# jeff-regier/Celeste.jl

Measured on AMD Instinct MI355X. Metric: sources/sec (ELBO value+gradient+Hessian+KL per target source), higher is better.
Workload: dtype f64; 1 GPU; BASELINE.json configs[2]: synthetic 2048x1489x5 SDSS-size field, 2000 star+galaxy sources, fp64, Sa=1 with value-only neighbours, psf_K=2; gather_backend=none, neighbor_links_rank0=3526

## Files before the change

### __graft_entry__.py

```python
import os
import subprocess
import sys

ROOT = os.path.dirname(os.path.abspath(__file__))
CSRC = os.path.join(ROOT, "celeste.jl_amd", "csrc")
LIB = os.path.join(CSRC, "libceleste_mi355x.so")
HIPCC = os.environ.get("HIPCC", "/opt/rocm/bin/hipcc")
HIP_FLAGS = ["--offload-arch=gfx950", "-O3", "-std=c++17", "-fPIC", "-shared", "-Wl,--version-script=exports.map"]
LINK_FLAGS = ["-L/opt/rocm/lib", "-lrccl", "-lpthread"]
DETECT_DIR = os.path.join(CSRC, "detect")
DETECT_LIB = os.path.join(DETECT_DIR, "libceleste_detect.so")
MCMC_DIR = os.path.join(CSRC, "mcmc")
MCMC_LIB = os.path.join(MCMC_DIR, "libceleste_mcmc.so")
BLEND_DIR = os.path.join(CSRC, "blend")
BLEND_LIB = os.path.join(BLEND_DIR, "libceleste_blend.so")
SYNTH_DIR = os.path.join(CSRC, "synth")
SYNTH_LIB = os.path.join(SYNTH_DIR, "libceleste_synth.so")


def _stale(target, sources):
    if not os.path.exists(target):
        return True
    t = os.path.getmtime(target)
    return any(os.path.getmtime(s) > t for s in sources)


def build() -> None:
    srcs = [os.path.join(CSRC, f) for f in os.listdir(CSRC) if f.endswith((".hip", ".h", ".inc", ".map"))]
    srcs.append(os.path.join(ROOT, "include", "celeste_mi355x.h"))
    srcs.append(os.path.abspath(__file__))
    if _stale(LIB, srcs):
        subprocess.check_call([HIPCC] + HIP_FLAGS + ["-o", LIB, os.path.join(CSRC, "celeste_abi.hip")] + LINK_FLAGS, cwd=CSRC)
    dsrcs = [os.path.join(DETECT_DIR, f) for f in os.listdir(DETECT_DIR) if f.endswith((".hip", ".h", ".map"))]
    dsrcs += [os.path.join(ROOT, "include", "celeste_detect.h"), os.path.abspath(__file__)]
    if _stale(DETECT_LIB, dsrcs):
        subprocess.check_call([HIPCC] + HIP_FLAGS + ["-o", DETECT_LIB, os.path.join(DETECT_DIR, "celeste_detect.hip"), "-lpthread"],
                              cwd=DETECT_DIR)
    msrcs = [os.path.join(MCMC_DIR, f) for f in os.listdir(MCMC_DIR) if f.endswith((".hip", ".h", ".map"))]
    msrcs += [os.path.join(CSRC, f) for f in os.listdir(CSRC) if f.endswith((".h", ".inc"))]
    msrcs += [os.path.join(ROOT, "include", "celeste_mcmc.h"), os.path.join(ROOT, "include", "celeste_mi355x.h"),
              os.path.abspath(__file__)]
    if _stale(MCMC_LIB, msrcs):
        subprocess.check_call([HIPCC] + HIP_FLAGS + ["-o", MCMC_LIB, os.path.join(MCMC_DIR, "celeste_mcmc.hip"), "-lpthread"],
                              cwd=MCMC_DIR)
    bsrcs = [os.path.join(BLEND_DIR, f) for f in os.listdir(BLEND_DIR) if f.endswith((".hip", ".h", ".map"))]
    bsrcs += [os.path.join(CSRC, f) for f in os.listdir(CSRC) if f.endswith((".hip", ".h", ".inc"))]
    bsrcs += [os.path.join(ROOT, "include", "celeste_blend.h"), os.path.join(ROOT, "include", "celeste_mi355x.h"),
              os.path.abspath(__file__)]
    if _stale(BLEND_LIB, bsrcs):
        subprocess.check_call([HIPCC] + HIP_FLAGS + ["-o", BLEND_LIB, os.path.join(BLEND_DIR, "celeste_blend.hip")] + LINK_FLAGS,
                              cwd=BLEND_DIR)
    ssrcs = [os.path.join(SYNTH_DIR, f) for f in os.listdir(SYNTH_DIR) if f.endswith((".hip", ".h", ".map"))]
    ssrcs += [os.path.join(CSRC, f) for f in os.listdir(CSRC) if f.endswith((".h", ".inc"))]
    ssrcs += [os.path.join(ROOT, "include", "celeste_synth.h"), os.path.join(ROOT, "include", "celeste_mi355x.h"),
              os.path.abspath(__file__)]
    if _stale(SYNTH_LIB, ssrcs):
        subprocess.check_call([HIPCC] + HIP_FLAGS + ["-o", SYNTH_LIB, os.path.join(SYNTH_DIR, "celeste_synth.hip"), "-lpthread"],
                              cwd=SYNTH_DIR)
    subprocess.check_call(["make", "-s", "-C", os.path.join(ROOT, "oracle")])
    fake_src, fake_lib = os.path.join(ROOT, "tests", "fake_rccl.c"), os.path.join(ROOT, "tests", "libfake_rccl.so")
    if _stale(fake_lib, [fake_src]):
        subprocess.check_call(["gcc", "-O2", "-fPIC", "-shared", "-Wall", "-D__HIP_PLATFORM_AMD__", "-I/opt/rocm/include", fake_src, "-o", fake_lib,
                               "-L/opt/rocm/lib", "-lamdhip64", "-lpthread", "-Wl,-rpath,/opt/rocm/lib"])
    if ROOT not in sys.path:
        sys.path.insert(0, ROOT)
    import celeste_jl_amd
    from celeste_jl_amd import cabi
    lib = cabi.load_library()
    for name in cabi.EXPORTED_SYMBOLS:
        getattr(lib, name)
    from celeste_jl_amd import detect
    dlib = detect.load_library()
    for name in detect.EXPORTED_SYMBOLS:
        getattr(dlib, name)
    from celeste_jl_amd import mcmc
    mlib = mcmc.load_library()
    for name in mcmc.EXPORTED_SYMBOLS:
        getattr(mlib, name)
    from celeste_jl_amd import blend
    blib = blend.load_library()
    for name in blend.EXPORTED_SYMBOLS:
        getattr(blib, name)
    from celeste_jl_amd import synth
    slib = synth.load_library()
    for name in synth.EXPORTED_SYMBOLS:
        getattr(slib, name)


def smoke() -> None:
    if ROOT not in sys.path:
        sys.path.insert(0, ROOT)
    import numpy as np
    import celeste_jl_amd as cel
    from celeste_jl_amd import synthetic, cabi
    from oracle import oracle
    f = synthetic.make_sample_dataset("two_body", seed=1)
    ctx = cel.FieldContext(f.images, f.patches, f.neighbors)
    v, d, h, cnt, st = ctx.eval_batch(f.vp, [0, 1])
    ov, od, oh, ocnt, ost = oracle.elbo_batch(ctx.problem, f.vp, [0, 1], n_threads=1)
    assert (st == 0).all() and (ost == 0).all()
    assert np.array_equal(cnt, ocnt), (cnt, ocnt)
    for a, b, name in ((v, ov, "v"), (d, od, "d"), (h, oh, "h")):
        scale = np.abs(b).max()
        err = np.abs(a - b).max() / scale
        assert err < 1e-8, (name, err)
    print("smoke ok: elbo =", v, "max rel err vs oracle < 1e-8")


if __name__ == "__main__":
    build()
    if len(sys.argv) > 1 and sys.argv[1] == "smoke":
        smoke()
```

### celeste.jl_amd/cabi.py

```python
import ctypes as C
import os
from typing import List, Optional, Sequence

import numpy as np

P = 44
STAMP = 51
COEF = 53

OK, ERR_INVALID_ARG, ERR_NONFINITE_INPUT, ERR_NONFINITE_RESULT, ERR_HIP, ERR_NO_DEVICE, ERR_ALLOC, ERR_ABORTED = range(8)
FLAG_GRAD, FLAG_HESS, FLAG_KL, FLAG_FP32, FLAG_SPLIT, FLAG_PACKED_HESS = 1, 2, 4, 8, 16, 32
HP = 990

_HERE = os.path.dirname(os.path.abspath(__file__))
LIB_PATH = os.path.join(_HERE, "csrc", "libceleste_mi355x.so")

c_double_p = C.POINTER(C.c_double)
c_float_p = C.POINTER(C.c_float)
c_int32_p = C.POINTER(C.c_int32)
c_int64_p = C.POINTER(C.c_int64)
c_uint8_p = C.POINTER(C.c_uint8)


class ImageT(C.Structure):
    _fields_ = [("H", C.c_int32), ("W", C.c_int32), ("band", C.c_int32), ("reserved", C.c_int32),
                ("pixels", c_float_p), ("sky", c_float_p), ("nelec_per_nmgy", c_float_p)]


class PatchT(C.Structure):
    _fields_ = [("off_h", C.c_int32), ("off_w", C.c_int32), ("H2", C.c_int32), ("W2", C.c_int32),
                ("bitmap", c_uint8_p), ("wcs_jacobian", C.c_double * 4), ("world_center", C.c_double * 2),
                ("pixel_center", C.c_double * 2), ("psf", c_double_p), ("stamp", C.c_int32),
                ("reserved", C.c_int32)]


class PriorT(C.Structure):
    _fields_ = [("is_star", C.c_double * 2), ("flux_mean", C.c_double * 2), ("flux_var", C.c_double * 2),
                ("k", (C.c_double * 8) * 2), ("color_mean", ((C.c_double * 4) * 8) * 2),
                ("color_cov", ((C.c_double * 16) * 8) * 2), ("gal_radius_px_mean", C.c_double),
                ("gal_radius_px_var", C.c_double)]


class ProblemT(C.Structure):
    _fields_ = [("n_images", C.c_int32), ("n_sources", C.c_int32), ("psf_K", C.c_int32), ("n_stamps", C.c_int32),
                ("images", C.POINTER(ImageT)), ("patches", C.POINTER(PatchT)), ("stamps", c_double_p),
                ("nbr_offsets", c_int64_p), ("nbr_index", c_int32_p), ("prior", C.POINTER(PriorT)),
                ("n_patch_entries", C.c_int64), ("patch_source", c_int32_p), ("patch_image", c_int32_p)]


class WorkStatsT(C.Structure):
    _fields_ = [("n_targets", C.c_int64), ("active_pixel_visits", C.c_int64), ("patch_rows", C.c_int64),
                ("neighbor_links", C.c_int64), ("algorithmic_bytes", C.c_int64), ("record_bytes", C.c_int64),
                ("record_tiles", C.c_int64)]


class OptimConfigT(C.Structure):
    _fields_ = [("loc_width", C.c_double), ("loc_scale", C.c_double), ("max_iters", C.c_int32),
                ("include_kl", C.c_int32), ("xtol_abs", C.c_double), ("ftol_rel", C.c_double), ("gtol", C.c_double),
                ("initial_delta", C.c_double), ("delta_hat", C.c_double), ("tr_secular_iters", C.c_int32),
                ("reserved", C.c_int32)]


class GroupInfoT(C.Structure):
    _fields_ = [("n_members", C.c_int32), ("n_devices", C.c_int32), ("exchange", C.c_int32), ("rccl_ranks", C.c_int32),
                ("devices", C.c_int32 * 16)]


EXCHANGE_RCCL, EXCHANGE_PEER_COPY = 1, 2


class CelesteError(RuntimeError):
    def __init__(self, status: int, msg: str):
        super().__init__("celeste_mi355x status %d: %s" % (status, msg))
        self.status = status


EXPORTED_SYMBOLS = [
    "celeste_version", "celeste_strerror", "celeste_ctx_create", "celeste_ctx_destroy", "celeste_elbo_eval",
    "celeste_elbo_eval_batch", "celeste_elbo_eval_multi", "celeste_elbo_eval_batch_device", "celeste_ctx_enable_timing",
    "celeste_ctx_last_kernel_ms", "celeste_ctx_last_record_sum_ms", "celeste_ctx_work_stats", "celeste_spline_prefilter",
    "celeste_ctx_spline_coefficients", "celeste_psf_raster",
    "celeste_maximize_batch", "celeste_render_expected", "celeste_optim_stats", "celeste_tr_solve_batch",
    "celeste_images_create", "celeste_images_destroy", "celeste_ctx_create_on",
    "celeste_host_alloc", "celeste_host_free", "celeste_host_register", "celeste_host_unregister",
    "celeste_maximize_batch_device", "celeste_joint_infer",
    "celeste_group_create", "celeste_group_destroy", "celeste_group_info", "celeste_group_elbo_eval_batch",
    "celeste_group_sweep_plan", "celeste_group_sweep", "celeste_group_sweep_wait", "celeste_group_sweep_results",
    "celeste_group_shard_sizes", "celeste_group_enable_timing", "celeste_group_last_sweep_ms", "celeste_group_last_kernel_ms",
    "celeste_group_maximize_batch", "celeste_group_joint_infer", "celeste_group_collectives",
]
ABI_VERSION = 220

_lib = None


def load_library(path: Optional[str] = None) -> C.CDLL:
    global _lib
    if _lib is not None and path is None:
        return _lib
    path = path or os.environ.get("CELESTE_MI355X_LIB") or LIB_PATH
    if not os.path.exists(path):
        raise ImportError(
            "HIP extension %s is missing: build it with `python -c 'import __graft_entry__ as g; g.build()'` "
            "(hipcc --offload-arch=gfx950). There is no CPU fallback." % path)
    try:
        import torch
        if torch.cuda.is_available():
            torch.cuda.init()
    except ImportError:
        pass
    except RuntimeError:
        pass
    lib = C.CDLL(path)
    vp = C.c_void_p
    lib.celeste_version.restype = C.c_int
    if lib.celeste_version() // 100 != ABI_VERSION // 100:
        raise ImportError("%s has ABI version %d, this binding was written against %d: the struct layouts "
                          "(celeste_optim_config_t ...) may differ -- rebuild the library" % (path, lib.celeste_version(), ABI_VERSION))
    lib.celeste_strerror.restype = C.c_char_p
    lib.celeste_strerror.argtypes = [C.c_int]
    lib.celeste_ctx_create.argtypes = [C.POINTER(ProblemT), C.c_int, C.POINTER(vp)]
    lib.celeste_ctx_destroy.argtypes = [vp]
    lib.celeste_ctx_destroy.restype = None
    lib.celeste_elbo_eval.argtypes = [vp, c_double_p, C.c_int32, C.c_uint32, c_double_p, c_double_p, c_double_p,
                                      c_int64_p, c_int64_p]
    lib.celeste_elbo_eval_batch.argtypes = [vp, c_double_p, C.c_int32, c_int32_p, C.c_uint32, c_double_p,
                                            c_double_p, c_double_p, c_int64_p, c_int32_p]
    lib.celeste_elbo_eval_batch_device.argtypes = [vp, vp, C.c_int32, vp, C.c_uint32, vp, vp, vp, vp, vp, vp]
    lib.celeste_ctx_enable_timing.argtypes = [vp, C.c_int]
    lib.celeste_ctx_last_kernel_ms.argtypes = [vp, C.POINTER(C.c_float)]
    lib.celeste_elbo_eval_multi.argtypes = [vp, c_double_p, C.c_int32, c_int32_p, C.c_uint32, C.POINTER(C.c_double),
                                            c_double_p, c_double_p, C.POINTER(C.c_int64), C.POINTER(C.c_int64)]
    lib.celeste_ctx_last_record_sum_ms.argtypes = [vp, C.POINTER(C.c_float)]
    lib.celeste_ctx_work_stats.argtypes = [vp, C.c_int32, c_int32_p, C.POINTER(WorkStatsT)]
    lib.celeste_spline_prefilter.argtypes = [c_double_p, c_double_p]
    lib.celeste_ctx_spline_coefficients.argtypes = [vp, C.c_int32, c_double_p]
    lib.celeste_psf_raster.argtypes = [C.c_int, c_double_p, C.c_int32, c_double_p, C.c_int32, c_double_p,
                                       C.c_int32, c_double_p]
    lib.celeste_maximize_batch.argtypes = [vp, c_double_p, c_double_p, c_double_p, C.c_int32, c_int32_p,
                                           C.POINTER(OptimConfigT), c_int32_p, c_int32_p, c_double_p, c_int32_p]
    lib.celeste_maximize_batch_device.argtypes = [vp, vp, vp, vp, C.c_int32, vp, C.POINTER(OptimConfigT), vp, vp, vp, vp, vp]
    lib.celeste_joint_infer.argtypes = [vp, c_double_p, C.c_int32, c_int64_p, c_int32_p, c_double_p,
                                        C.POINTER(OptimConfigT), c_int32_p, c_int32_p, c_double_p, c_int32_p]
    lib.celeste_optim_stats.argtypes = [C.c_int, C.POINTER(C.c_uint64)]
    lib.celeste_tr_solve_batch.argtypes = [C.c_int, C.c_int32, c_double_p, c_double_p, c_double_p, C.c_int32, C.c_int32,
                                           c_double_p, c_double_p, c_int32_p, c_int32_p]
    lib.celeste_render_expected.argtypes = [vp, c_double_p, C.c_int32, c_double_p]
    lib.celeste_images_create.argtypes = [C.c_int32, C.POINTER(ImageT), C.c_int, C.POINTER(vp)]
    lib.celeste_images_destroy.argtypes = [vp]
    lib.celeste_images_destroy.restype = None
    lib.celeste_ctx_create_on.argtypes = [vp, C.POINTER(ProblemT), C.POINTER(vp)]
    lib.celeste_host_alloc.argtypes = [C.c_size_t]
    lib.celeste_host_alloc.restype = vp
    lib.celeste_host_free.argtypes = [vp]
    lib.celeste_host_free.restype = None
    lib.celeste_host_register.argtypes = [vp, C.c_size_t]
    lib.celeste_host_unregister.argtypes = [vp]
    c_float_p_ = C.POINTER(C.c_float)
    lib.celeste_group_create.argtypes = [C.POINTER(ProblemT), C.c_int32, c_int32_p, C.POINTER(vp)]
    lib.celeste_group_destroy.argtypes = [vp]
    lib.celeste_group_destroy.restype = None
    lib.celeste_group_info.argtypes = [vp, C.POINTER(GroupInfoT)]
    lib.celeste_group_collectives.argtypes = [vp, c_int64_p, c_int32_p]
    lib.celeste_group_elbo_eval_batch.argtypes = [vp, c_double_p, C.c_int32, c_int32_p, C.c_uint32, c_double_p, c_double_p,
                                                  c_double_p, c_int64_p, c_int32_p]
    lib.celeste_group_sweep_plan.argtypes = [vp, c_double_p, C.c_int32, c_int32_p, C.c_uint32]
    lib.celeste_group_sweep.argtypes = [vp]
    lib.celeste_group_sweep_wait.argtypes = [vp]
    lib.celeste_group_sweep_results.argtypes = [vp, c_double_p, c_double_p, c_double_p, c_int64_p, c_int32_p]
    lib.celeste_group_shard_sizes.argtypes = [vp, c_int32_p, c_int64_p]
    lib.celeste_group_enable_timing.argtypes = [vp, C.c_int]
    lib.celeste_group_last_sweep_ms.argtypes = [vp, c_float_p_, c_float_p_]
    lib.celeste_group_last_kernel_ms.argtypes = [vp, C.c_int32, c_float_p_]
    lib.celeste_group_maximize_batch.argtypes = [vp, c_double_p, c_double_p, c_double_p, C.c_int32, c_int32_p,
                                                 C.POINTER(OptimConfigT), c_int32_p, c_int32_p, c_double_p, c_int32_p]
    lib.celeste_group_joint_infer.argtypes = [vp, c_double_p, C.c_int32, C.c_int32, c_int64_p, c_int64_p, c_int32_p, c_double_p,
                                              C.POINTER(OptimConfigT), c_int32_p, c_int32_p, c_double_p, c_int32_p, c_int64_p]
    _lib = lib
    return lib


def check(status: int, lib=None):
    if status != OK:
        lib = lib or load_library()
        raise CelesteError(status, lib.celeste_strerror(status).decode())


def _dp(a: np.ndarray):
    return a.ctypes.data_as(c_double_p)


def marshal_image_structs(images, keep: list):
    c_images = (ImageT * len(images))()
    for n, im in enumerate(images):
        pix = np.asfortranarray(im.pixels, dtype=np.float32)
        sky = np.asfortranarray(im.sky, dtype=np.float32)
        iota = np.ascontiguousarray(im.nelec_per_nmgy, dtype=np.float32)
        assert sky.shape == pix.shape and iota.shape == (pix.shape[0],)
        keep += [pix, sky, iota]
        ci = c_images[n]
        ci.H, ci.W, ci.band = pix.shape[0], pix.shape[1], int(im.b)
        ci.pixels = pix.ctypes.data_as(c_float_p)
        ci.sky = sky.ctypes.data_as(c_float_p)
        ci.nelec_per_nmgy = iota.ctypes.data_as(c_float_p)
    return c_images


class ImageSet:

    def __init__(self, images, device: int = 0):
        self.lib = load_library()
# ... 288 lines not shown
```

### celeste.jl_amd/csrc/celeste_abi.hip

```cpp
#include <hip/hip_runtime.h>
#include <algorithm>
#include <atomic>
#include <cmath>
#include <cstdio>
#include <cstdlib>
#include <cstring>
#include <mutex>
#include <unordered_map>
#include <vector>

#include "elbo_kernels.h"
#include "optim_kernels.h"
#include "fused_kernels.h"
#include "host_tables.h"

struct celeste_group;

#define EVAL_FUSED_MAX 32

#define HIP_TRY(expr)                                                                    \
    do {                                                                                 \
        hipError_t e__ = (expr);                                                         \
        if (e__ != hipSuccess) {                                                         \
            fprintf(stderr, "celeste_mi355x: %s failed: %s (%s:%d)\n", #expr,            \
// ... 49 lines not shown
    static const size_t cap = [] { const char *v = getenv("CELESTE_PINNED_POOL_KB"); return (size_t)(v ? std::max(0, atoi(v)) : 16384) << 10; }();
    return cap;
}
static hipError_t staging_alloc(void **p, size_t bytes) {
    *p = nullptr;
    int k = -1;
    if (pinned_pool_cap() && bytes <= (1u << 20)) { k = 0; while (((size_t)4096 << k) < bytes) ++k; }
    if (k < 0) return hipHostMalloc(p, std::max<size_t>(bytes, 1), hipHostMallocPortable);
    PinnedPool &pp = pinned_pool();
    {
        std::lock_guard<std::mutex> lk(pp.mu);
        if (!pp.idle[k].empty()) { *p = pp.idle[k].back(); pp.idle[k].pop_back(); pp.idle_bytes -= (size_t)4096 << k; pp.live[*p] = k; return hipSuccess; }
    }
    hipError_t e = hipHostMalloc(p, (size_t)4096 << k, hipHostMallocPortable);
    if (e == hipSuccess) { std::lock_guard<std::mutex> lk(pp.mu); pp.live[*p] = k; }
    return e;
}
static void staging_free(void *p) {
    if (!p) return;
    {
        PinnedPool &pp = pinned_pool();
        std::lock_guard<std::mutex> lk(pp.mu);
        auto it = pp.live.find(p);
        if (it != pp.live.end()) {
            const int k = it->second;
            pp.live.erase(it);
            if (pp.idle_bytes + ((size_t)4096 << k) <= pinned_pool_cap()) { pp.idle[k].push_back(p); pp.idle_bytes += (size_t)4096 << k; return; }
        }
    }
    (void)hipHostFree(p);
}


struct celeste_images {
    int device = 0;
    int N = 0;
    std::vector<DevImage> h_images;
    std::vector<void *> plane_allocs;
    DevImage *d_images = nullptr;
    std::atomic<int> refs{1};
};

static void images_release(celeste_images *im) {
    if (!im || im->refs.fetch_sub(1) != 1) return;
    (void)hipSetDevice(im->device);
    for (void *p : im->plane_allocs) (void)hipFree(p);
    if (im->d_images) (void)hipFree(im->d_images);
    delete im;
}

struct celeste_ctx {
    int device = 0;
    celeste_images *imgs = nullptr;
    hipStream_t stream = nullptr;
    hipStream_t copy_stream = nullptr;
    bool copy_stream_checked = false;
    int N = 0, S = 0, K = 0, NC = 0, n_stamps = 0;
    int chunk_px = 256, CH = 1;
    int max_npx = 0;
    std::vector<DevPatch> h_patches;
    std::vector<int64_t> h_nbr_off;
    std::vector<int32_t> h_nbr_idx;
    DevImage *d_images = nullptr;
    DevPatch *d_patches = nullptr;
    double *d_coefs = nullptr;
    float *d_coefs_f = nullptr;
    uint8_t *d_bitmaps = nullptr;
    int64_t *d_nbr_off = nullptr;
    int32_t *d_nbr_idx = nullptr;
    PriorDev *d_prior = nullptr;
    SrcImg *d_srcimg = nullptr;
    Comp *d_comps = nullptr;
    SrcGeo *d_geo = nullptr;
    int64_t *d_val_off = nullptr;
    double2 *d_val = nullptr;
    int32_t *d_needed = nullptr;
    int32_t stamp = 0;
    std::vector<int32_t> h_vis_off, h_vis_img, h_vis_src;
    int32_t *d_vis_off = nullptr, *d_vis_img = nullptr, *d_vis_src = nullptr;
    int4 *d_value_items = nullptr;
    int4 *d_vitems_src = nullptr;
    int32_t *d_vitem_off = nullptr;
    std::vector<int32_t> h_vitem_off;
    int64_t n_value_items = 0;
    int32_t *d_prep_mark = nullptr;
    double *d_lg_sum = nullptr;
    int64_t *d_nv_base = nullptr;
    int32_t *d_nbr_vis = nullptr;
    int2 *d_items = nullptr;
    size_t items_cap = 0;
    std::vector<int32_t> h_src_chunks;
    std::vector<int64_t> h_top_chunks;
    int max_src_chunks = 0;
    int32_t *d_work = nullptr, *d_work_blk = nullptr, *d_work_total = nullptr;
    size_t work_cap = 0, work_blk_cap = 0;
    int M = 1;
    bool dense = false;
    int64_t V = 0;
    std::vector<int64_t> h_tile_off;
    int64_t *d_tile_off = nullptr;
    int64_t n_tiles = 0;
    int sum_tiles = 4, RCH = 1;
    double *d_rec = nullptr;
    double *d_acc_split = nullptr;
    size_t acc_split_cap = 0;
    double *d_acc = nullptr;
    size_t acc_cap = 0;
    int32_t *d_rec_off = nullptr;
    size_t rec_off_cap = 0;
    double *d_vp = nullptr;
    int32_t *d_targets = nullptr;
    double *d_v = nullptr, *d_d = nullptr, *d_h = nullptr;
    int64_t *d_cnt = nullptr;
    int32_t *d_status = nullptr;
    size_t stage_cap = 0;
    double *p_vp = nullptr;
    int32_t *p_targets = nullptr, *p_status = nullptr;
    double *p_v = nullptr, *p_d = nullptr, *p_h = nullptr;
    int64_t *p_cnt = nullptr;
    size_t pin_cap = 0;
    double *d_small_in = nullptr, *p_small_in = nullptr, *d_small_out = nullptr, *p_small_out = nullptr;
    static const int MAX_PARTS = 8;
    hipEvent_t part_done[MAX_PARTS] = {}, part_copied[MAX_PARTS] = {};
    struct OptBuffers {
        size_t cap = 0;
        double *d_vp = nullptr, *d_v = nullptr, *d_d = nullptr, *d_h = nullptr, *d_H = nullptr, *d_T = nullptr, *d_S = nullptr, *d_pos = nullptr;
        int32_t *d_targets = nullptr, *d_act[2] = {nullptr, nullptr}, *d_evt[2] = {nullptr, nullptr}, *d_count = nullptr,
                *d_st = nullptr;
        void *d_state = nullptr;
        static const int RING = 4;
        double *h_vp = nullptr;
        void *h_state = nullptr;
        int32_t *h_count = nullptr;
        hipEvent_t ev[RING] = {};
    } opt;
    struct FusedBuffers {
        size_t cap_t = 0, cap_rec = 0, cap_q = 0, cap_saved = 0;
        bool arrivals_dirty = true;
        int4 *d_chunk_desc = nullptr;
        int2 *d_tgt_rec = nullptr;
        int32_t *d_q_items = nullptr, *d_q_ctl = nullptr, *d_arrivals = nullptr;
        double *d_saved = nullptr;
        int32_t *h_ctl = nullptr;
        int max_resident = 0;
        int cus = 0;
    } fused;
    struct Scratch { void *p = nullptr; size_t cap = 0; } scratch[24];
    int timing = 0;
    hipEvent_t ev[5] = {nullptr, nullptr, nullptr, nullptr, nullptr};
    int ev_split = 0;
    int ev_valid = 0;
};

#define ABI_CATCH catch (const std::bad_alloc &) { return CELESTE_ERR_ALLOC; } catch (...) { return CELESTE_ERR_HIP; }

extern "C" int celeste_version(void) { return CELESTE_ABI_VERSION; }

extern "C" const char *celeste_strerror(int status) {
    switch (status) {
        case CELESTE_OK: return "ok";
        case CELESTE_ERR_INVALID_ARG: return "invalid argument";
        case CELESTE_ERR_NONFINITE_INPUT: return "vp contains NaNs or Infs";
        case CELESTE_ERR_NONFINITE_RESULT: return "ELBO value, gradient or Hessian contains Inf/NaNs";
        case CELESTE_ERR_HIP: return "HIP runtime error";
        case CELESTE_ERR_NO_DEVICE: return "no HIP device (the engine has no CPU fallback)";
        case CELESTE_ERR_ALLOC: return "allocation failed";
        case CELESTE_ERR_ABORTED: return "device group aborted: a member failed in front of a collective (destroy the group and create it again)";
// ... 277 lines not shown
        CTX_TRY(dev_upload(&c->d_val_off, voff.data(), voff.size()));
        CTX_TRY(dev_upload<double2>(&c->d_val, nullptr, (size_t)tot));
        CTX_TRY(dev_upload<int32_t>(&c->d_needed, nullptr, (size_t)c->S));
        if (hipMemset(c->d_needed, 0, (size_t)c->S * sizeof(int32_t)) != hipSuccess) { celeste_ctx_destroy(c); return CELESTE_ERR_HIP; }
    }

    CTX_TRY(dev_upload(&c->d_vis_off, c->h_vis_off.data(), c->h_vis_off.size()));
    CTX_TRY(dev_upload(&c->d_vis_img, c->h_vis_img.data(), c->h_vis_img.size()));
    CTX_TRY(dev_upload(&c->d_vis_src, c->h_vis_src.data(), c->h_vis_src.size()));
    CTX_TRY(dev_upload<double>(&c->d_lg_sum, nullptr, (size_t)c->V));
    if (c->V > 0)
        hipLaunchKernelGGL(patch_lgamma_kernel, dim3((unsigned)c->V), dim3(256), 0, nullptr, c->d_images, c->d_patches,
                           c->d_vis_img, c->d_bitmaps, c->d_lg_sum);
    const char *env_chunk = getenv("CELESTE_CHUNK_PX");
    if (env_chunk && atoi(env_chunk) >= 64) c->chunk_px = (atoi(env_chunk) + 63) / 64 * 64;
    c->CH = c->max_npx > 0 ? (c->max_npx + c->chunk_px - 1) / c->chunk_px : 1;
    c->h_src_chunks.assign((size_t)c->S, 0);
    for (int s = 0; s < c->S; ++s) {
        for (int v = c->h_vis_off[s]; v < c->h_vis_off[s + 1]; ++v) {
            const DevPatch &q = c->h_patches[v];
            c->h_src_chunks[s] += (q.H2 * q.W2 + c->chunk_px - 1) / c->chunk_px;
        }
        c->max_src_chunks = std::max(c->max_src_chunks, c->h_src_chunks[s]);
    }
    auto hv = [c](int s, int n) -> int64_t {
        if (c->dense) return (int64_t)s * c->N + n;
        const int32_t *b = c->h_vis_img.data() + c->h_vis_off[s], *e = c->h_vis_img.data() + c->h_vis_off[s + 1];
        const int32_t *it = std::lower_bound(b, e, n);
        return it != e && *it == n ? (int64_t)(it - c->h_vis_img.data()) : -1;
    };
    if (!c->dense) {
        std::vector<int64_t> base((size_t)c->S + 1, 0);
        for (int s = 0; s < c->S; ++s)
            base[s + 1] = base[s] + (int64_t)(c->h_vis_off[s + 1] - c->h_vis_off[s]) * (c->h_nbr_off[s + 1] - c->h_nbr_off[s]);
        std::vector<int32_t> nv((size_t)base[c->S]);
        for (int s = 0; s < c->S; ++s) {
            const int64_t K = c->h_nbr_off[s + 1] - c->h_nbr_off[s];
            for (int v = c->h_vis_off[s]; v < c->h_vis_off[s + 1]; ++v)
                for (int64_t q = 0; q < K; ++q)
                    nv[base[s] + (int64_t)(v - c->h_vis_off[s]) * K + q] = (int32_t)hv(c->h_nbr_idx[c->h_nbr_off[s] + q], c->h_vis_img[v]);
        }
        CTX_TRY(dev_upload(&c->d_nv_base, base.data(), base.size()));
        CTX_TRY(dev_upload(&c->d_nbr_vis, nv.data(), nv.size()));
    }
    {
        std::vector<int32_t> sorted(c->h_src_chunks);
        std::sort(sorted.begin(), sorted.end(), [](int32_t a, int32_t b) { return a > b; });
        c->h_top_chunks.assign((size_t)c->S + 1, 0);
        for (int s = 0; s < c->S; ++s) c->h_top_chunks[s + 1] = c->h_top_chunks[s] + sorted[s];
    }
    CTX_TRY(dev_upload<int32_t>(&c->d_work_total, nullptr, 1));
    {
        if (c->N > 0xffff) { celeste_ctx_destroy(c); return CELESTE_ERR_INVALID_ARG; }
        const int n_cls = c->chunk_px / 64;
        std::vector<std::vector<std::pair<int32_t, int32_t>>> by_len(n_cls);
        for (int s = 0; s < c->S; ++s)
            for (int64_t q = c->h_nbr_off[s]; q < c->h_nbr_off[s + 1]; ++q) {
                const int s2 = c->h_nbr_idx[q];
                for (int va = c->h_vis_off[s]; va < c->h_vis_off[s + 1]; ++va) {
                    const int n = c->h_vis_img[va];
                    const int64_t vb = hv(s2, n);
                    if (vb < 0) continue;
                    const DevPatch &a = c->h_patches[va], &b = c->h_patches[vb];
                    const int rh = std::min(a.off_h + a.H2, b.off_h + b.H2) - std::max(a.off_h, b.off_h);
                    const int rw = std::min(a.off_w + a.W2, b.off_w + b.W2 - 1) - std::max(a.off_w, b.off_w);
                    if (rh <= 0 || rw <= 0) continue;
                    const int npx = rh * rw, nch = (npx + c->chunk_px - 1) / c->chunk_px;
                    for (int ch = 0; ch < nch; ++ch) {
                        const int px = std::min(c->chunk_px, npx - ch * c->chunk_px);
                        by_len[n_cls - (px + 63) / 64].push_back({(int32_t)q, (int32_t)(n | (ch << 16))});
                    }
                }
            }
        std::vector<int32_t> link_src(c->h_nbr_idx.size());
        for (int s = 0; s < c->S; ++s)
            for (int64_t q = c->h_nbr_off[s]; q < c->h_nbr_off[s + 1]; ++q) link_src[q] = s;
        std::vector<int4> desc;
        for (auto &v : by_len)
            for (auto &e : v) {
                const int t = link_src[e.first], s2 = c->h_nbr_idx[e.first], n = e.second & 0xffff, ch = e.second >> 16;
                desc.push_back(make_int4((int)hv(s2, n), (int)hv(t, n), ch, t));
            }
        c->n_value_items = (int64_t)desc.size();
        CTX_TRY(dev_upload(&c->d_value_items, desc.data(), desc.size()));
        c->h_vitem_off.assign((size_t)c->S + 1, 0);
        for (auto &d : desc) c->h_vitem_off[(size_t)d.w + 1]++;
        for (int s = 0; s < c->S; ++s) c->h_vitem_off[s + 1] += c->h_vitem_off[s];
        {
            std::vector<int4> by_src(desc.size());
            std::vector<int32_t> fill(c->h_vitem_off.begin(), c->h_vitem_off.end() - 1);
            for (auto &d : desc) by_src[(size_t)fill[d.w]++] = d;
            CTX_TRY(dev_upload(&c->d_vitems_src, by_src.data(), by_src.size()));
            CTX_TRY(dev_upload(&c->d_vitem_off, c->h_vitem_off.data(), c->h_vitem_off.size()));
        }
        CTX_TRY(dev_upload<int32_t>(&c->d_prep_mark, nullptr, (size_t)c->S));
        if (hipMemset(c->d_prep_mark, 0, (size_t)c->S * sizeof(int32_t)) != hipSuccess) { celeste_ctx_destroy(c); return CELESTE_ERR_HIP; }
    }
    {
        c->h_tile_off.resize(c->h_patches.size());
        int64_t tot = 0;
        for (size_t q = 0; q < c->h_patches.size(); ++q) {
            c->h_tile_off[q] = tot;
            tot += ((int64_t)c->h_patches[q].H2 * c->h_patches[q].W2 + 63) / 64;
        }
        c->n_tiles = tot;
        if (const char *e = getenv("CELESTE_SUM_TILES")) if (atoi(e) > 0) c->sum_tiles = atoi(e);
        c->RCH = std::max(1, ((c->max_npx + 63) / 64 + c->sum_tiles - 1) / c->sum_tiles);
    }
    if (hipStreamSynchronize(nullptr) != hipSuccess) { celeste_ctx_destroy(c); return CELESTE_ERR_HIP; }
#undef CTX_TRY
    *out = c;
    return CELESTE_OK;
} ABI_CATCH

extern "C" void celeste_ctx_destroy(celeste_ctx_t *c) {
    if (!c) return;
    (void)hipSetDevice(c->device);
    if (c->stream) (void)hipStreamSynchronize(c->stream);
    if (c->copy_stream) (void)hipStreamSynchronize(c->copy_stream);
    void *ptrs[] = {c->d_patches, c->d_coefs, c->d_coefs_f, c->d_bitmaps, c->d_nbr_off, c->d_nbr_idx, c->d_prior,
                    c->d_srcimg, c->d_comps, c->d_geo, c->d_val_off, c->d_val, c->d_needed, c->d_vis_off, c->d_vis_img, c->d_vis_src, c->d_value_items, c->d_vitems_src, c->d_vitem_off, c->d_prep_mark, c->d_rec_off, c->d_lg_sum, c->d_nv_base, c->d_nbr_vis, c->d_items, c->d_work, c->d_work_blk, c->d_work_total, c->d_tile_off, c->d_rec, c->d_acc_split, c->d_acc, c->d_vp, c->d_targets, c->d_v, c->d_d, c->d_h,
                    c->d_cnt, c->d_status};
    for (void *p : ptrs) if (p) (void)hipFree(p);
    {
        auto &o = c->opt;
        void *optr[] = {o.d_vp, o.d_v, o.d_d, o.d_h, o.d_H, o.d_T, o.d_S, o.d_pos, o.d_targets, o.d_act[0], o.d_act[1], o.d_evt[0], o.d_evt[1],
                        o.d_count, o.d_st, o.d_state};
        for (void *q : optr) if (q) (void)hipFree(q);
        void *hptr[] = {o.h_vp, o.h_state, o.h_count};
        for (void *q : hptr) if (q) staging_free(q);
        for (int k = 0; k < celeste_ctx::OptBuffers::RING; ++k) if (o.ev[k]) (void)hipEventDestroy(o.ev[k]);
        auto &f = c->fused;
        void *fptr[] = {f.d_chunk_desc, f.d_tgt_rec, f.d_q_items, f.d_q_ctl, f.d_arrivals, f.d_saved};
        for (void *q : fptr) if (q) (void)hipFree(q);
        if (f.h_ctl) staging_free(f.h_ctl);
    }
    for (auto &sc : c->scratch) if (sc.p) (void)hipFree(sc.p);
    for (int i = 0; i < 5; ++i) if (c->ev[i]) (void)hipEventDestroy(c->ev[i]);
    for (int i = 0; i < celeste_ctx::MAX_PARTS; ++i) {
        if (c->part_done[i]) (void)hipEventDestroy(c->part_done[i]);
        if (c->part_copied[i]) (void)hipEventDestroy(c->part_copied[i]);
    }
    void *pins[] = {c->p_vp, c->p_targets, c->p_status, c->p_v, c->p_d, c->p_h, c->p_cnt, c->p_small_in, c->p_small_out};
    if (c->d_small_in) (void)hipFree(c->d_small_in);
    if (c->d_small_out) (void)hipFree(c->d_small_out);
    for (void *q : pins) if (q) staging_free(q);
    stream_retire(c->device, c->stream);
    stream_retire(c->device, c->copy_stream);
    images_release(c->imgs);
    delete c;
}

template <class T>
static hipError_t scratch_get(celeste_ctx_t *c, int k, size_t bytes, T **out) {
    auto &s = c->scratch[k];
    if (bytes > s.cap) {
        hipError_t e = s.p ? hipStreamSynchronize(c->stream) : hipSuccess;
        if (e != hipSuccess) return e;
        if (s.p) { (void)hipFree(s.p); s.p = nullptr; s.cap = 0; }
        e = hipMalloc(&s.p, std::max<size_t>(bytes, 256));
        if (e != hipSuccess) return e;
        s.cap = std::max<size_t>(bytes, 256);
    }
    *out = (T *)s.p;
    return hipSuccess;
}

static int launch_eval(celeste_ctx_t *c, const double *d_vp, int32_t n_targets, const int32_t *d_targets,
                       uint32_t flags, double *d_v, double *d_d, double *d_h, int64_t *d_counters, int32_t *d_status,
                       void *stream_, bool render_neighbors, const int32_t *d_active_rank = nullptr,
                       int64_t n_chunks = -1, bool tables_current = false, const int32_t *d_live = nullptr,
                       bool prep_all = false, bool render_only = false, const int32_t *d_h_pos = nullptr);

extern "C" int celeste_elbo_eval_batch_device(celeste_ctx_t *c, const double *d_vp, int32_t n_targets,
                                              const int32_t *d_targets, uint32_t flags, double *d_v, double *d_d,
                                              double *d_h, int64_t *d_counters, int32_t *d_status, void *stream_) try {
    return launch_eval(c, d_vp, n_targets, d_targets, flags, d_v, d_d, d_h, d_counters, d_status, stream_, true);
} ABI_CATCH

static int ensure_part_events(celeste_ctx_t *c, int n) {
    for (int k = 0; k < n && k < celeste_ctx::MAX_PARTS; ++k) {
        if (!c->part_done[k]) HIP_TRY(hipEventCreateWithFlags(&c->part_done[k], hipEventDisableTiming));
        if (!c->part_copied[k]) HIP_TRY(hipEventCreateWithFlags(&c->part_copied[k], hipEventDisableTiming));
    }
    return CELESTE_OK;
}

static void fused_args_tables(celeste_ctx_t *c, FusedArgs &A) {
    A.images = c->d_images; A.patches = c->d_patches; A.coefs = c->d_coefs; A.bitmaps = c->d_bitmaps;
    A.nbr_off = c->d_nbr_off; A.nbr_idx = c->d_nbr_idx; A.val_off = c->d_val_off; A.val = c->d_val;
    A.nv_base = c->d_nv_base; A.nbr_vis = c->d_nbr_vis; A.items = c->dense ? nullptr : c->d_items; A.geo = c->d_geo;
    A.prior = c->d_prior; A.vis_off = c->d_vis_off; A.vis_img = c->d_vis_img; A.lg_sum = c->d_lg_sum; A.rec_off = c->d_rec_off;
    A.N = c->N; A.NC = c->NC; A.K = c->K; A.M = c->M; A.CH = c->CH; A.chunk_px = c->chunk_px;
    A.acc = c->d_acc;
    A.st = nullptr; A.Hstate = nullptr; A.Tstate = nullptr; A.Spec = nullptr; A.q_items = nullptr; A.q_ctl = nullptr; A.q_cap = 0; A.timeout_ticks = 0;
    A.j_R = 0; A.j_gshift = 0; A.j_dep = nullptr; A.j_succ_off = nullptr; A.j_succ = nullptr; A.j_vitem_off = nullptr;
    A.j_vitems = nullptr; A.j_render_arr = nullptr; A.j_saved = nullptr; A.j_pos = nullptr; A.j_srcimg = nullptr;
    A.j_comps = nullptr; A.j_geo = nullptr;
}

static int fused_buffers(celeste_ctx_t *c, size_t n, size_t rec, hipStream_t stream) {
    auto &fb = c->fused;
    if (n > fb.cap_t) {
        if (fb.d_tgt_rec || fb.d_arrivals) HIP_TRY(hipStreamSynchronize(stream));
        void **ps[] = {(void **)&fb.d_tgt_rec, (void **)&fb.d_arrivals};
        for (void **q : ps) if (*q) { (void)hipFree(*q); *q = nullptr; }
        fb.cap_t = 0;
        HIP_TRY(hipMalloc((void **)&fb.d_tgt_rec, n * sizeof(int2)));
        HIP_TRY(hipMalloc((void **)&fb.d_arrivals, n * sizeof(int32_t)));
        fb.cap_t = n;
        fb.arrivals_dirty = true;
    }
    if (rec > fb.cap_rec) {
        if (fb.d_chunk_desc) { HIP_TRY(hipStreamSynchronize(stream)); (void)hipFree(fb.d_chunk_desc); fb.d_chunk_desc = nullptr; }
        fb.cap_rec = 0;
        HIP_TRY(hipMalloc((void **)&fb.d_chunk_desc, std::max<size_t>(rec, 1) * 2 * sizeof(int4)));
        fb.cap_rec = rec;
    }
    return CELESTE_OK;
}

#define VALUE_WIDE_MAX 768
static int launch_eval(celeste_ctx_t *c, const double *d_vp, int32_t n_targets, const int32_t *d_targets,
                       uint32_t flags, double *d_v, double *d_d, double *d_h, int64_t *d_counters, int32_t *d_status,
                       void *stream_, bool render_neighbors, const int32_t *d_active_rank, int64_t n_chunks,
                       bool tables_current, const int32_t *d_live, bool prep_all, bool render_only, const int32_t *d_h_pos) {
    if (!c || !d_vp || !d_targets || !d_v || !d_status || n_targets < 0) return CELESTE_ERR_INVALID_ARG;
    if ((flags & CELESTE_FLAG_HESS) && !d_h) return CELESTE_ERR_INVALID_ARG;
    if ((flags & (CELESTE_FLAG_GRAD | CELESTE_FLAG_HESS)) && !d_d) return CELESTE_ERR_INVALID_ARG;
    if (n_targets == 0) return CELESTE_OK;
    hipStream_t stream = (hipStream_t)stream_;
    HIP_TRY(hipSetDevice(c->device));
    const bool big_chunks = (flags & CELESTE_FLAG_FP32) && !(flags & CELESTE_FLAG_SPLIT) && !d_active_rank && c->chunk_px == 256 &&
                            !getenv("CELESTE_FP32_CHUNK_256");
    const int chunk_px = big_chunks ? 512 : c->chunk_px;
    const int CH = big_chunks ? std::max(1, (c->max_npx + chunk_px - 1) / chunk_px) : c->CH;
    const size_t rec_cap = n_chunks >= 0 ? (size_t)n_chunks
                                         : std::min((size_t)n_targets * c->max_src_chunks, (size_t)n_targets * c->M * c->CH);
    const size_t need = std::max<size_t>(rec_cap, 1) * ACC_N;
    if ((size_t)n_targets * c->M > c->rec_off_cap) {
        if (c->d_rec_off) { HIP_TRY(hipStreamSynchronize(stream)); HIP_TRY(hipFree(c->d_rec_off)); c->d_rec_off = nullptr; }
        HIP_TRY(hipMalloc((void **)&c->d_rec_off, (size_t)n_targets * c->M * sizeof(int32_t)));
        c->rec_off_cap = (size_t)n_targets * c->M;
    }
    if (need > c->acc_cap) {
        if (c->d_acc) { HIP_TRY(hipStreamSynchronize(stream)); HIP_TRY(hipFree(c->d_acc)); c->d_acc = nullptr; }
        HIP_TRY(hipMalloc((void **)&c->d_acc, need * sizeof(double)));
        c->acc_cap = need;
    }
    if (!c->dense && (size_t)n_targets * c->M > c->items_cap) {
        if (c->d_items) { HIP_TRY(hipStreamSynchronize(stream)); HIP_TRY(hipFree(c->d_items)); c->d_items = nullptr; }
        HIP_TRY(hipMalloc((void **)&c->d_items, (size_t)n_targets * c->M * sizeof(int2)));
        c->items_cap = (size_t)n_targets * c->M;
    }
    const int n_visits = n_targets * c->M;
    const int n_wblk = (n_visits + WORK_NT - 1) / WORK_NT;
    const size_t work_need = (size_t)(n_chunks >= 0 ? n_chunks : (int64_t)n_targets * c->max_src_chunks);
    const size_t grid_need = (size_t)(n_chunks >= 0 ? n_chunks
                                      : n_targets <= c->S ? c->h_top_chunks[n_targets] : (int64_t)n_targets * c->max_src_chunks);
    if ((size_t)n_targets * c->M * c->CH > 0x7fffffffull) return CELESTE_ERR_INVALID_ARG;
    if (work_need > c->work_cap) {
        if (c->d_work) { HIP_TRY(hipStreamSynchronize(stream)); HIP_TRY(hipFree(c->d_work)); c->d_work = nullptr; }
        HIP_TRY(hipMalloc((void **)&c->d_work, std::max<size_t>(work_need, 1) * sizeof(int32_t)));
        c->work_cap = work_need;
    }
    int G = n_targets >= 8192 ? 4 : n_targets >= 768 ? 2 : 1;
    if (const char *e = getenv("CELESTE_CHUNK_GROUP")) if (atoi(e) >= 1 && atoi(e) <= 16) G = atoi(e);
    bool eval_fused = !render_only && (flags & CELESTE_FLAG_HESS) && !(flags & (CELESTE_FLAG_FP32 | CELESTE_FLAG_SPLIT)) &&
                      !d_active_rank && !d_live && !d_h_pos && d_d && d_h && n_targets <= EVAL_FUSED_MAX;
    if (const char *e = getenv("CELESTE_EVAL_FUSED")) {
        if (atoi(e) == 0) eval_fused = false;
        else if (atoi(e) == 1) eval_fused = !render_only && (flags & CELESTE_FLAG_HESS) && !(flags & (CELESTE_FLAG_FP32 | CELESTE_FLAG_SPLIT)) &&
                                          !d_active_rank && !d_live && !d_h_pos && d_d && d_h;
    }
    if (eval_fused) G = 1;
    const int n_classes = WORK_CLASSES;
    if ((size_t)n_wblk * (n_classes + 1) > c->work_blk_cap) {
        if (c->d_work_blk) { HIP_TRY(hipStreamSynchronize(stream)); HIP_TRY(hipFree(c->d_work_blk)); c->d_work_blk = nullptr; }
        HIP_TRY(hipMalloc((void **)&c->d_work_blk, (size_t)n_wblk * (n_classes + 1) * sizeof(int32_t)));
        c->work_blk_cap = (size_t)n_wblk * (n_classes + 1);
    }
    const bool derivs = (flags & (CELESTE_FLAG_GRAD | CELESTE_FLAG_HESS)) != 0;
    const bool split = (flags & CELESTE_FLAG_SPLIT) != 0;
    if (split) {
        if (!(flags & CELESTE_FLAG_HESS)) return CELESTE_ERR_INVALID_ARG;
        if (!c->d_rec) {
            HIP_TRY(hipStreamSynchronize(stream));
            if (dev_upload(&c->d_tile_off, c->h_tile_off.data(), c->h_tile_off.size()) != CELESTE_OK) return CELESTE_ERR_HIP;
            if (hipMalloc((void **)&c->d_rec, (size_t)std::max<int64_t>(c->n_tiles, 1) * ACC_N * 64 * sizeof(double)) != hipSuccess)
                return CELESTE_ERR_ALLOC;
        }
        const size_t need_s = (size_t)n_targets * c->M * c->RCH * ACC_N;
        if (need_s > c->acc_split_cap) {
            if (c->d_acc_split) { HIP_TRY(hipStreamSynchronize(stream)); HIP_TRY(hipFree(c->d_acc_split)); c->d_acc_split = nullptr; }
            HIP_TRY(hipMalloc((void **)&c->d_acc_split, need_s * sizeof(double)));
            c->acc_split_cap = need_s;
        }
    }
    if (c->timing) HIP_TRY(hipEventRecord(c->ev[0], stream));
    if (render_neighbors && ++c->stamp == 0x7fffffff) {
        HIP_TRY(hipMemsetAsync(c->d_needed, 0, (size_t)c->S * sizeof(int32_t), stream));
        c->stamp = 1;
    }
    const int geo_S = render_neighbors ? c->S : -1;
    const size_t setup_threads = std::max<size_t>(render_neighbors ? (size_t)c->S : 0, (size_t)n_targets * (c->dense ? 1 : c->M));
    int32_t *const prep_mark = render_neighbors && !tables_current && !prep_all ? c->d_prep_mark : nullptr;
    bool prep_fused = false;
    bool records_described = false;
    if (eval_fused) { int stb = fused_buffers(c, (size_t)n_targets, rec_cap, stream); if (stb != CELESTE_OK) return stb; }
    if (n_visits <= WORK1_MAX_VISITS && !getenv("CELESTE_PARALLEL_WORKLIST")) {
        const unsigned setup_blocks = (unsigned)((setup_threads + WORK1_SETUP - 1) / WORK1_SETUP);
        prep_fused = !render_neighbors && !getenv("CELESTE_NO_FUSED_PREP");
        const bool prep_all_here = render_neighbors && !tables_current && c->V > 0 && c->V <= WORK1_PREP_ALL_MAX &&
                                   (n_targets >= WORK1_PREP_ALL_MIN_TARGETS || c->V <= WORK1_PREP_ALL_TINY) && !getenv("CELESTE_NO_FUSED_PREP");
        const int prep_n = prep_all_here ? (int)c->V : n_visits;
        if (prep_all_here) prep_fused = true;
        const unsigned prep_blocks = prep_fused ? (unsigned)((prep_n + WORK1_NT / 64 - 1) / (WORK1_NT / 64)) : 0u;
        const bool records_described_here = eval_fused && c->dense && !d_live && !getenv("CELESTE_NO_FUSED_DESCRIBE");
        hipLaunchKernelGGL(setup_worklist_kernel, dim3(1 + setup_blocks + prep_blocks), dim3(WORK1_NT),
                           0, stream, d_vp, geo_S, c->d_geo, d_targets, n_targets, c->d_vis_off, c->d_vis_img, c->M,
                           c->dense ? nullptr : c->d_items, render_neighbors ? c->d_needed : nullptr, c->stamp, c->d_patches,
                           c->N, CH, chunk_px, G, (int)c->dense, c->d_work, c->d_work_total, d_live, prep_mark,
                           c->d_nbr_off, c->d_nbr_idx, c->d_rec_off, (int)setup_blocks, c->d_images, c->K, c->d_srcimg,
                           c->d_comps, prep_all_here ? (int)c->V : 0, c->d_vis_src,
                           records_described_here ? c->fused.d_chunk_desc : nullptr, records_described_here ? c->fused.d_tgt_rec : nullptr,
                           c->chunk_px);
        records_described = records_described_here;
    } else {
        hipLaunchKernelGGL(setup_kernel, dim3((unsigned)((setup_threads + 63) / 64)), dim3(64), 0, stream, d_vp, geo_S,
                           c->d_geo, d_targets, n_targets, c->d_vis_off, c->d_vis_img, c->M, c->dense ? nullptr : c->d_items,
                           render_neighbors ? c->d_needed : nullptr, c->stamp, prep_mark, c->d_nbr_off, c->d_nbr_idx, d_live);
        hipLaunchKernelGGL(work_count_kernel, dim3(n_wblk), dim3(WORK_NT), 0, stream, d_targets, n_visits, c->d_patches,
                           c->d_vis_off, c->d_vis_img, c->N, c->M, chunk_px, G, (int)c->dense, c->d_work_blk, d_live);
        hipLaunchKernelGGL(work_scan_kernel, dim3(1), dim3(1024), 0, stream, c->d_work_blk, n_wblk * (n_classes + 1),
                           c->d_work_total, n_wblk * n_classes);
        hipLaunchKernelGGL(work_fill_kernel, dim3(n_wblk), dim3(WORK_NT), 0, stream, d_targets, n_visits, c->d_patches,
                           c->d_vis_off, c->d_vis_img, c->N, c->M, CH, chunk_px, G, (int)c->dense, c->d_work_blk, c->d_work, d_live,
                           c->d_rec_off);
    }
    if (render_neighbors) {
        if (c->V > 0 && !tables_current && !prep_fused)
            hipLaunchKernelGGL(prep_kernel, dim3((unsigned)c->V), dim3(64), 0, stream, d_vp, c->d_images, c->d_patches,
                               c->d_vis_src, c->d_vis_img, c->N, c->K, c->d_srcimg, c->d_comps, nullptr, c->d_vis_off, c->M,
                               (int)c->dense, nullptr, prep_mark, c->stamp);
    } else if (!prep_fused) {
        hipLaunchKernelGGL(prep_kernel, dim3((unsigned)std::max(n_visits, 1)), dim3(64), 0, stream, d_vp, c->d_images,
                           c->d_patches, c->d_vis_src, c->d_vis_img, c->N, c->K, c->d_srcimg, c->d_comps, d_targets,
                           c->d_vis_off, c->M, (int)c->dense, d_live, nullptr, 0);
    }
    if (render_neighbors) {
    if (c->n_value_items > 0)
    {
        const bool wide_items = n_targets <= VALUE_WIDE_MAX && c->chunk_px == 256 && !getenv("CELESTE_NO_WIDE_VALUE");
#define LAUNCH_VALUE(R, WAVES)                                                                                              \
        hipLaunchKernelGGL((value_kernel<R, WAVES>), dim3((unsigned)c->n_value_items), dim3(64 * WAVES), 0, stream,       \
                           c->d_patches, c->d_coefs, c->d_srcimg, c->d_comps, c->d_needed, c->stamp, c->d_val_off,          \
                           c->d_value_items, c->NC, c->chunk_px, c->d_val, c->d_coefs_f)
        if (flags & CELESTE_FLAG_FP32) { if (wide_items) LAUNCH_VALUE(float, 2); else LAUNCH_VALUE(float, 1); }
        else { if (wide_items) LAUNCH_VALUE(double, 4); else LAUNCH_VALUE(double, 1); }
#undef LAUNCH_VALUE
    }
    }
    if (render_only) { HIP_TRY(hipGetLastError()); return CELESTE_OK; }
    if (c->timing) HIP_TRY(hipEventRecord(c->ev[1], stream));
    if (eval_fused) {
        auto &fb = c->fused;
        if (fb.arrivals_dirty) {
            HIP_TRY(hipMemsetAsync(fb.d_arrivals, 0, fb.cap_t * sizeof(int32_t), stream));
            fb.arrivals_dirty = false;
        }
        if (!records_described)
            hipLaunchKernelGGL(fused_setup_kernel, dim3((unsigned)((n_targets + 63) / 64)), dim3(64), 0, stream, d_targets, n_targets,
                               c->d_patches, c->d_vis_off, c->dense ? nullptr : c->d_items, c->N, c->M, c->chunk_px, c->d_rec_off,
                               fb.d_chunk_desc, fb.d_tgt_rec, (int32_t *)nullptr, (int32_t *)nullptr);
        FusedArgs A;
        fused_args_tables(c, A);
        A.targets = d_targets; A.n_targets = n_targets; A.vp = const_cast<double *>(d_vp);
        A.chunk_desc = fb.d_chunk_desc; A.tgt_rec = fb.d_tgt_rec; A.arrivals = fb.d_arrivals; A.flags = flags;
        memset(&A.op, 0, sizeof A.op);
        const unsigned rec_bound = (unsigned)std::max<size_t>(n_chunks >= 0 ? grid_need : work_need, 1);
        hipLaunchKernelGGL(eval_fused_kernel, dim3(rec_bound + (unsigned)n_targets), dim3(FUSED_NT), 0, stream, A, c->d_srcimg,
                           c->d_comps, c->d_work_total, (int)rec_bound, d_v, d_d, d_h, d_counters, d_status);
        if (c->timing) { HIP_TRY(hipEventRecord(c->ev[2], stream)); HIP_TRY(hipEventRecord(c->ev[3], stream)); c->ev_valid = 1; c->ev_split = 0; }
        HIP_TRY(hipGetLastError());
        return CELESTE_OK;
    }
    const dim3 grid((unsigned)std::max<size_t>(grid_need, 1));
#define PIXEL_ARGS                                                                                                \
    c->d_images, c->d_patches, c->d_coefs, c->d_bitmaps, c->d_srcimg, c->d_comps, c->d_nbr_off, c->d_nbr_idx,       \
    c->d_val_off, c->d_val, d_targets, c->N, c->NC, CH, chunk_px, G, c->d_acc, c->d_tile_off, c->d_rec, \
    d_active_rank, c->d_items, c->M, c->d_work, c->d_work_total, c->d_nv_base, c->d_nbr_vis, c->d_rec_off, c->d_coefs_f
#define LAUNCH_PIXEL_T(MODE, R) hipLaunchKernelGGL((pixel_kernel<MODE, R>), grid, dim3(64), 0, stream, PIXEL_ARGS)
#define LAUNCH_PIXEL_M(MODE) hipLaunchKernelGGL((pixel_kernel<MODE, double, true>), grid, dim3(64), 0, stream, PIXEL_ARGS)
#define LAUNCH_PIXEL(MODE) do { if (flags & CELESTE_FLAG_FP32) LAUNCH_PIXEL_T(MODE, float); else LAUNCH_PIXEL_T(MODE, double); } while (0)
    if (d_active_rank) {
        if (flags & CELESTE_FLAG_HESS) LAUNCH_PIXEL_M(2);
        else if (derivs) LAUNCH_PIXEL_M(1);
        else LAUNCH_PIXEL_M(0);
    }
    else if (split) LAUNCH_PIXEL(3);
    else if (flags & CELESTE_FLAG_HESS) LAUNCH_PIXEL(2);
    else if (derivs) LAUNCH_PIXEL(1);
    else LAUNCH_PIXEL_T(0, double);
#undef LAUNCH_PIXEL
#undef LAUNCH_PIXEL_M
#undef PIXEL_ARGS
#undef LAUNCH_PIXEL_T
    if (c->timing) HIP_TRY(hipEventRecord(c->ev[2], stream));
    c->ev_split = 0;
    const int lift_nt = n_targets <= 1024 ? 512 : 256;
    bool lift7 = n_targets > 4096;
    if (const char *e = getenv("CELESTE_LIFT_WAVES")) lift7 = atoi(e) == 7;
#define LAUNCH_LIFT(...) do { if (lift7) hipLaunchKernelGGL(lift_kernel<7>, __VA_ARGS__); else hipLaunchKernelGGL(lift_kernel<8>, __VA_ARGS__); } while (0)
    if (split) {
        hipLaunchKernelGGL(record_sum_kernel, dim3((unsigned)((size_t)n_targets * c->M * c->RCH)), dim3(RSUM_NT), 0,
                           stream, c->d_patches, d_targets, c->d_tile_off, reinterpret_cast<const double2 *>(c->d_rec),
                           c->d_items, c->N, c->M, c->RCH, c->sum_tiles, c->d_acc_split, nullptr, c->d_work_total);
        if (c->timing) { HIP_TRY(hipEventRecord(c->ev[4], stream)); c->ev_split = 1; }
        LAUNCH_LIFT(dim3(n_targets), dim3(lift_nt), 0, stream, d_vp, c->d_images, c->d_patches, c->d_geo,
                           c->d_nbr_off, c->d_nbr_idx, d_targets, c->d_acc_split, c->d_prior, c->d_vis_off, c->d_vis_img, c->N, c->M,
                           c->RCH, c->sum_tiles * 64, flags,
                           d_v, d_d, d_h, d_counters, d_status, d_live, d_active_rank ? nullptr : c->d_lg_sum, nullptr, d_h_pos);
    } else
    LAUNCH_LIFT(dim3(n_targets), dim3(lift_nt), 0, stream, d_vp, c->d_images, c->d_patches, c->d_geo,
                       c->d_nbr_off, c->d_nbr_idx, d_targets, c->d_acc, c->d_prior, c->d_vis_off, c->d_vis_img, c->N, c->M, CH,
                       chunk_px, flags,
                       d_v, d_d, d_h, d_counters, d_status, d_live, d_active_rank ? nullptr : c->d_lg_sum, c->d_rec_off, d_h_pos);
#undef LAUNCH_LIFT
    if (c->timing) { HIP_TRY(hipEventRecord(c->ev[3], stream)); c->ev_valid = 1; }
    HIP_TRY(hipGetLastError());
    return CELESTE_OK;
}

__global__ void spin_kernel(long long ticks) {
    const long long t0 = wall_clock64();
    while (wall_clock64() - t0 < ticks) __builtin_amdgcn_s_sleep(8);
}
static int pick_copy_stream(celeste_ctx_t *c) {
    if (c->copy_stream_checked) return CELESTE_OK;
    c->copy_stream_checked = true;
    if (const char *e = getenv("CELESTE_COPY_STREAM_CHECK")) if (atoi(e) == 0) return CELESTE_OK;
    const size_t bytes = 4u << 20;
    void *d_buf = nullptr, *h_buf = nullptr;
    hipEvent_t e0 = nullptr, e1 = nullptr;
    if (hipMalloc(&d_buf, bytes) != hipSuccess || hipHostMalloc(&h_buf, bytes, hipHostMallocDefault) != hipSuccess ||
        hipEventCreate(&e0) != hipSuccess || hipEventCreate(&e1) != hipSuccess) {
        (void)hipGetLastError();
        if (d_buf) (void)hipFree(d_buf);
        if (h_buf) (void)hipHostFree(h_buf);
        if (e0) (void)hipEventDestroy(e0);
        if (e1) (void)hipEventDestroy(e1);
        return CELESTE_OK;
    }
    const float spin_ms = 0.3f;
    auto measure = [&](hipStream_t s, float *ms) -> bool {
        if (hipEventRecord(e0, c->stream) != hipSuccess) return false;
        hipLaunchKernelGGL(spin_kernel, dim3(1), dim3(64), 0, c->stream, (long long)(spin_ms * 1e5));
        if (hipStreamWaitEvent(s, e0, 0) != hipSuccess || hipMemcpyAsync(h_buf, d_buf, bytes, hipMemcpyDeviceToHost, s) != hipSuccess ||
            hipEventRecord(e1, s) != hipSuccess || hipStreamSynchronize(s) != hipSuccess || hipStreamSynchronize(c->stream) != hipSuccess)
            return false;
        return hipEventElapsedTime(ms, e0, e1) == hipSuccess;
    };
    float best = 0;
    hipStream_t retired[3]; int n_retired = 0;
    bool ok = measure(c->copy_stream, &best) && measure(c->copy_stream, &best);
    for (int k = 0; ok && best > spin_ms && k < 3; ++k) {
        hipStream_t s = nullptr;
        float ms = 0;
        if (stream_acquire(c->device, &s) != hipSuccess) break;
        if (measure(s, &ms) && measure(s, &ms) && ms < best) { std::swap(s, c->copy_stream); best = ms; }
        retired[n_retired++] = s;
    }
    for (int k = 0; k < n_retired; ++k) stream_retire(c->device, retired[k]);
    (void)hipGetLastError();
    (void)hipFree(d_buf); (void)hipHostFree(h_buf); (void)hipEventDestroy(e0); (void)hipEventDestroy(e1);
    return CELESTE_OK;
}

extern "C" void *celeste_host_alloc(size_t bytes) {
    void *p = nullptr;
    if (hipHostMalloc(&p, std::max<size_t>(bytes, 1), hipHostMallocDefault) != hipSuccess) { (void)hipGetLastError(); return nullptr; }
    return p;
}
extern "C" void celeste_host_free(void *ptr) { if (ptr) (void)hipHostFree(ptr); }
extern "C" int celeste_host_register(void *ptr, size_t bytes) try {
    if (!ptr || bytes == 0) return CELESTE_ERR_INVALID_ARG;
    if (hipHostRegister(ptr, bytes, hipHostRegisterDefault) != hipSuccess) { (void)hipGetLastError(); return CELESTE_ERR_HIP; }
    return CELESTE_OK;
} ABI_CATCH
extern "C" int celeste_host_unregister(void *ptr) try {
    if (!ptr) return CELESTE_ERR_INVALID_ARG;
    if (hipHostUnregister(ptr) != hipSuccess) { (void)hipGetLastError(); return CELESTE_ERR_HIP; }
    return CELESTE_OK;
} ABI_CATCH
static bool is_pinned(const void *ptr, size_t bytes) {
    if (!ptr || bytes == 0) return false;
    hipPointerAttribute_t a;
    if (hipPointerGetAttributes(&a, ptr) != hipSuccess) { (void)hipGetLastError(); return false; }
    if (a.type != hipMemoryTypeHost) return false;
    if (hipPointerGetAttributes(&a, (const char *)ptr + bytes - 1) != hipSuccess) { (void)hipGetLastError(); return false; }
    return a.type == hipMemoryTypeHost;
}

template <class T>
static int pinned_grow(T **p, size_t n) {
    if (*p) { staging_free(*p); *p = nullptr; }
    HIP_TRY(staging_alloc((void **)p, std::max<size_t>(n, 1) * sizeof(T)));
    return CELESTE_OK;
}

#define EVAL_SMALL_MAX 32
static int eval_small(celeste_ctx_t *c, const double *vp, int32_t n_targets, const int32_t *targets, uint32_t flags, double *v,
                      double *d, double *h, int64_t *counters, int32_t *status) {
    const size_t n = (size_t)n_targets, HS = (flags & CELESTE_FLAG_PACKED_HESS) ? CELESTE_HP : (size_t)CEL_P * CEL_P;
    const size_t vp_n = (size_t)c->S * CEL_P;
// ... 962 lines not shown
```

### celeste.jl_amd/csrc/elbo_kernels.h

```cpp
#pragma once
#include <hip/hip_runtime.h>
#include <math.h>
#include "elbo_device.h"
#include "../../include/celeste_mi355x.h"

#ifndef CELESTE_MUTANT
#define CELESTE_MUTANT 0
#endif

__constant__ double c_eta[16];
__constant__ double c_nu[16];

__device__ inline void bvn_cov(double ab, double angle, double scale, double &x11, double &x12, double &x22) {
    double sp, cp;
    sincos(angle, &sp, &cp);
    double ab_term = ab * ab - 1.0;
    double s2 = scale * scale;
    x12 = -s2 * cp * sp * ab_term;
    x11 = s2 * (1.0 + ab_term * (sp * sp));
    x22 = s2 * (1.0 + ab_term * (cp * cp));
}

__device__ inline void brightness(const double *vs, int i, int b, double &El, double &Ell) {
    const double r = vs[6 + i], v = vs[8 + i];
// ... 19 lines not shown
}
template <bool MOMENTS = true>
__device__ __forceinline__ void prep_visit_values(int c, const double *__restrict__ vs, const DevPatch &p, int b, int K,
                                                  SrcImg *__restrict__ si_out, Comp *__restrict__ comps_out) {
    const int NC = 14 * K;
    double m1, m2;
    world_to_pix(vs, p, m1, m2);
    double x11, x12, x22;
    bvn_cov(vs[3], vs[4], vs[5], x11, x12, x22);
    if (c < NC) {
        int i, j, k;
        if (c < 8 * K) { i = 0; k = c / 8; j = c - 8 * k; }
        else { int cc = c - 8 * K; i = 1; k = cc / 6; j = cc - 6 * k; }
        const double *pc = p.psf + 6 * k;
        const double nu = c_nu[8 * i + j];
        const double s11 = pc[3] + nu * x11, s12 = pc[4] + nu * x12, s22 = pc[5] + nu * x22;
        const double det = s11 * s22 - s12 * s12;
        const double idet = 1.0 / det;
        const double z = (pc[0] * c_eta[8 * i + j]) / (sqrt(det) * (2.0 * M_PI));
        Comp o;
        o.p11 = s22 * idet; o.p12 = -s12 * idet; o.p22 = s11 * idet;
        o.xi1 = pc[1]; o.xi2 = pc[2];
        const double dev = vs[2];
        o.w0 = z * (i == 0 ? dev : 1.0 - dev);
        o.wd = (i == 0 ? z : -z);
        o.nu = nu;
        comps_out[c] = o;
    }
    if (MOMENTS && c == 63) {
        double El0, Ell0, El1, Ell1;
        brightness(vs, 0, b, El0, Ell0);
        brightness(vs, 1, b, El1, Ell1);
        SrcImg o;
        o.m1 = m1; o.m2 = m2;
        o.c0 = vs[26] * El0; o.c1 = vs[27] * El1;
        o.q0 = vs[26] * Ell0; o.q1 = vs[27] * Ell1;
        o.dev = vs[2]; o.pad1 = 0;
        *si_out = o;
    }
}

__device__ __forceinline__ void brightness_moments_wave(int lane, const double *__restrict__ vs, const DevPatch &p, int b,
                                                        SrcImg *__restrict__ si_out) {
    double fac = 1.0;
    if (lane < 20) {
        const int i = lane / 10, w = (lane / 5) & 1, f = lane % 5;
        const double r = vs[6 + i], v = vs[8 + i];
        const double *cm = vs + 10 + 4 * i, *cv = vs + 18 + 4 * i;
        const int col = f == 1 ? 2 : (f == 2 ? 3 : (f == 3 ? 1 : 0));
        const double sgn = f >= 3 ? -1.0 : 1.0;
        double arg;
        if (f == 0) arg = w ? 2 * r + 2 * v : r + 0.5 * v;
        else arg = w ? 2 * (sgn * cm[col]) + 2 * cv[col] : sgn * cm[col] + .5 * cv[col];
        fac = exp(arg);
    }
    const int base = lane < 4 ? 5 * lane : 0;
    double prod = __shfl(fac, base, 64);
    const double f1 = __shfl(fac, base + 1, 64), f2 = __shfl(fac, base + 2, 64), f3 = __shfl(fac, base + 3, 64),
                 f4 = __shfl(fac, base + 4, 64);
    if (b >= 3) prod *= f1;
    if (b >= 4) prod *= f2;
    if (b <= 1) prod *= f3;
    if (b <= 0) prod *= f4;
    const double El0 = __shfl(prod, 0, 64), Ell0 = __shfl(prod, 1, 64), El1 = __shfl(prod, 2, 64), Ell1 = __shfl(prod, 3, 64);
    if (lane == 0) {
        SrcImg o;
        world_to_pix(vs, p, o.m1, o.m2);
        o.c0 = vs[26] * El0; o.c1 = vs[27] * El1;
        o.q0 = vs[26] * Ell0; o.q1 = vs[27] * Ell1;
        o.dev = vs[2]; o.pad1 = 0;
        *si_out = o;
    }
}
__device__ __forceinline__ void prep_visit(int c, int s, int n, int sn, const double *__restrict__ vp,
                                           const DevImage *__restrict__ images, const DevPatch *__restrict__ patches, int K,
                                           SrcImg *__restrict__ srcimg, Comp *__restrict__ comps) {
    const double *vs = vp + (size_t)s * CEL_P;
    const DevPatch &p = patches[sn];
    const int b = images[n].band - 1;
    prep_visit_values<false>(c, vs, p, b, K, srcimg + sn, comps + (size_t)sn * (14 * K));
    brightness_moments_wave(c, vs, p, b, srcimg + sn);
}

__global__ void __launch_bounds__(64)
prep_kernel(const double *__restrict__ vp, const DevImage *__restrict__ images,
            const DevPatch *__restrict__ patches, const int32_t *__restrict__ vis_src,
            const int32_t *__restrict__ vis_img, int N, int K,
            SrcImg *__restrict__ srcimg, Comp *__restrict__ comps,
            const int32_t *__restrict__ targets, const int32_t *__restrict__ vis_off, int M, int dense,
            const int32_t *__restrict__ live, const int32_t *__restrict__ mark, int32_t stamp) {
    int s, n, sn;
    if (targets) {
        const int k = blockIdx.x, ti = k / M, j = k - ti * M;
        if (live && ti >= *live) return;
        s = targets[ti];
        n = j;
        if (!dense) {
            const int vo = vis_off[s];
            if (j >= vis_off[s + 1] - vo) return;
            n = vis_img[vo + j];
        }
        sn = dense ? s * N + n : vis_off[s] + j;
        const DevPatch &q = patches[sn];
        if (q.H2 * q.W2 <= 0) return;
    } else {
        s = vis_src[blockIdx.x]; n = vis_img[blockIdx.x];
        sn = blockIdx.x;
        if (mark && mark[s] != stamp) return;
    }
    prep_visit(threadIdx.x, s, n, sn, vp, images, patches, K, srcimg, comps);
}

__device__ __forceinline__ void source_geo_values(const double *vs, SrcGeo *out) {
    double x11, x12, x22;
    bvn_cov(vs[3], vs[4], vs[5], x11, x12, x22);
        SrcGeo g;
        const double ab = vs[3], ang = vs[4], r = vs[5];
        double sn_, cs_;
        sincos(ang, &sn_, &cs_);
        const double cos_sin = cs_ * sn_, sin_sq = sn_ * sn_, cos_sq = cs_ * cs_;
        const double r2 = r * r;
        double *j = g.jsh, *t = g.tsh;
        const double c1 = 2 * ab * r2;
        j[0] = c1 * sin_sq; j[1] = -c1 * cos_sin; j[2] = c1 * cos_sq;
        const double c2 = r2 * (ab * ab - 1);
        j[3] = c2 * (2 * cos_sin); j[4] = c2 * (sin_sq - cos_sq); j[5] = c2 * (-2 * cos_sin);
        j[6] = 2 * x11 / r; j[7] = 2 * x12 / r; j[8] = 2 * x22 / r;
        const double a = 2 * r2;
        t[0] = sin_sq * a; t[1] = -cos_sin * a; t[2] = cos_sq * a;
        t[3] = 2 * cos_sin * a * ab; t[4] = (sin_sq - cos_sq) * a * ab; t[5] = -2 * cos_sin * a * ab;
        t[6] = 2 * j[0] / r; t[7] = 2 * j[1] / r; t[8] = 2 * j[2] / r;
        t[9] = t[3]; t[10] = t[4]; t[11] = t[5];
        const double b2 = a * (ab * ab - 1);
        t[12] = (cos_sq - sin_sq) * b2; t[13] = 2 * cos_sin * b2; t[14] = (sin_sq - cos_sq) * b2;
        t[15] = 2 * j[3] / r; t[16] = 2 * j[4] / r; t[17] = 2 * j[5] / r;
        t[18] = t[6]; t[19] = t[7]; t[20] = t[8];
        t[21] = t[15]; t[22] = t[16]; t[23] = t[17];
        t[24] = 2 * x11 / r2; t[25] = 2 * x12 / r2; t[26] = 2 * x22 / r2;
        int fin = 1;
        for (int q = 0; q < CEL_P; ++q) fin &= (int)isfinite(vs[q]);
        g.finite = fin; g.pad = 0;
        *out = g;
}
__device__ inline void source_geo(const double *vp, int s, SrcGeo *geo) { source_geo_values(vp + (size_t)s * CEL_P, geo + s); }

__global__ void iota_kernel(const float *__restrict__ iota, int H, double *__restrict__ log_iota) {
    const int i = blockIdx.x * blockDim.x + threadIdx.x;
    if (i < H) log_iota[i] = (double)(float)log((double)iota[i]);
}
__global__ void __launch_bounds__(256)
patch_lgamma_kernel(const DevImage *__restrict__ images, const DevPatch *__restrict__ patches,
                    const int32_t *__restrict__ vis_img, const uint8_t *__restrict__ bitmaps, double *__restrict__ out) {
    __shared__ double s_part[256];
    const int v = blockIdx.x;
    const DevPatch &P = patches[v];
    const DevImage &img = images[vis_img[v]];
    const int npx = P.H2 * P.W2;
    double s = 0.0;
    for (int idx = threadIdx.x; idx < npx; idx += 256) {
        const int w2 = idx / P.H2, h2 = idx - w2 * P.H2;
        const float x = img.pixels[(size_t)(P.off_h + h2) + (size_t)img.H * (P.off_w + w2)];
        bool valid = !isnan(x);
        if (valid && P.bitmap_off >= 0) valid = bitmaps[P.bitmap_off + h2 + (int64_t)P.H2 * w2] != 0;
        if (valid) s += lgamma((double)x + 1.0);
    }
    s_part[threadIdx.x] = s;
    __syncthreads();
    for (int o = 128; o >= 1; o >>= 1) {
        if ((int)threadIdx.x < o) s_part[threadIdx.x] += s_part[threadIdx.x + o];
        __syncthreads();
    }
    if (threadIdx.x == 0) out[v] = s_part[0];
}

__device__ __forceinline__ void prefilter_line_dev(const double *__restrict__ d, int dstride, double *__restrict__ c, int cstride,
                                                   const double *__restrict__ cp) {
#pragma clang fp contract(off)
    constexpr int n = CEL_STAMP, m = CEL_STAMP - 2;
    const double x1 = d[0], xn = d[(n - 1) * dstride];
    double prev = 0.0;
    for (int q = 0; q < m; ++q) {
        double rhs = 6.0 * d[(q + 1) * dstride];
        if (q == 0) rhs -= x1;
        if (q == m - 1) rhs -= xn;
        const double lower = (q == 0) ? 0.0 : 1.0;
        const double denom = 4.0 - lower * (q ? cp[q - 1] : 0.0);
        prev = (rhs - lower * prev) / denom;
        c[(2 + q) * cstride] = prev;
    }
    double nxt = prev;
    for (int q = m - 2; q >= 0; --q) {
        nxt = c[(2 + q) * cstride] - cp[q] * nxt;
        c[(2 + q) * cstride] = nxt;
// ... 170 lines not shown
    float wx[4], wy[4];
    bspline_w(xh - (float)ix, wx); bspline_w(xw - (float)iy, wy);
    const double *c0 = coef + (ix - 1) + CEL_COEF * (iy - 1);
    float y = 0;
#pragma unroll
    for (int b = 0; b < 4; ++b) {
        const double *cb = c0 + CEL_COEF * b;
        const float r = (float)cb[0] * wx[0] + (float)cb[1] * wx[1] + (float)cb[2] * wx[2] + (float)cb[3] * wx[3];
        y += r * wy[b];
    }
    return y < 0 ? 1e-3f * __expf(y) : 1e-3f * (y + 1.0f);
}
typedef float vf2 __attribute__((ext_vector_type(2)));
__device__ inline float galaxy_value_f(const float *tcf, int NC, float dx, float dy) {
    const vf2 *tp = reinterpret_cast<const vf2 *>(tcf);
    const vf2 dxx = (vf2)(dx), dyy = (vf2)(dy);
    vf2 v = (vf2)(0.0f);
    for (int c = 0; c < NC; c += 2) {
        const vf2 *k = tp + 3 * c;
        const vf2 p11 = k[0], p12 = k[1], p22 = k[2], xi1 = k[3], xi2 = k[4], w0 = k[5];
        const vf2 d1 = dxx - xi1, d2 = dyy - xi2;
        const vf2 u = p11 * d1 + p12 * d2, vv = p12 * d1 + p22 * d2;
        const vf2 q = -0.5f * (d1 * u + d2 * vv);
        const vf2 e = {__expf(q.x), __expf(q.y)};
        v += w0 * e;
    }
    return v.x + v.y;
}

__device__ __forceinline__ void divmod_small(int idx, int d, float rd, int &q, int &r) {
    q = (int)((float)idx * rd);
    r = idx - q * d;
    if (r < 0) { --q; r += d; }
    else if (r >= d) { ++q; r -= d; }
}

__device__ inline double wave_sum(double x) {
#pragma unroll
    for (int o = 32; o >= 1; o >>= 1) x += __shfl_xor(x, o, 64);
    return x;
}

template <bool COH>
__device__ __forceinline__ double ldc(const double *p) {
    if constexpr (COH)
        return __builtin_bit_cast(double, __hip_atomic_load(reinterpret_cast<const unsigned long long *>(p), __ATOMIC_RELAXED,
                                                            __HIP_MEMORY_SCOPE_AGENT));
    else return *p;
}
template <bool COH>
__device__ __forceinline__ void stc(double *p, double v) {
    if constexpr (COH)
        __hip_atomic_store(reinterpret_cast<unsigned long long *>(p), __builtin_bit_cast(unsigned long long, v), __ATOMIC_RELAXED,
                           __HIP_MEMORY_SCOPE_AGENT);
    else *p = v;
}
template <bool COH>
__device__ __forceinline__ int ldc(const int *p) {
    if constexpr (COH) return __hip_atomic_load(p, __ATOMIC_RELAXED, __HIP_MEMORY_SCOPE_AGENT);
    else return *p;
}
template <bool COH>
__device__ __forceinline__ void stc(int *p, int v) {
    if constexpr (COH) __hip_atomic_store(p, v, __ATOMIC_RELAXED, __HIP_MEMORY_SCOPE_AGENT);
    else *p = v;
}


__device__ __forceinline__ int table_entry(const int32_t *__restrict__ vis_off, const int32_t *__restrict__ vis_img,
                                           int dense, int N, int s, int n) {
    if (dense) return s * N + n;
    for (int v = vis_off[s]; v < vis_off[s + 1]; ++v) if (vis_img[v] == n) return v;
    return -1;
}

__device__ inline void source_geo(const double *vp, int s, SrcGeo *geo);
__device__ inline void setup_thread(int k, const double *__restrict__ vp, int S, SrcGeo *__restrict__ geo,
                                    const int32_t *__restrict__ targets, int n_targets, const int32_t *__restrict__ vis_off,
                                    const int32_t *__restrict__ vis_img, int M, int2 *__restrict__ items,
                                    int32_t *__restrict__ is_target, int32_t stamp, int32_t *__restrict__ prep_mark,
                                    const int64_t *__restrict__ nbr_off, const int32_t *__restrict__ nbr_idx,
                                    const int32_t *__restrict__ live = nullptr) {
    if (live) n_targets = min(n_targets, *live);
    if (S < 0) { if (k < n_targets) source_geo(vp, targets[k], geo); }
    else if (k < S) source_geo(vp, k, geo);
    if (prep_mark && k < n_targets) {
        const int t = targets[k];
        prep_mark[t] = stamp;
        for (int64_t q = nbr_off[t]; q < nbr_off[t + 1]; ++q) prep_mark[nbr_idx[q]] = stamp;
    }
    if (items && k < n_targets * M) {
        const int ti = k / M, j = k - ti * M;
        const int t = targets[ti];
        const int vo = vis_off[t];
        items[k] = j < vis_off[t + 1] - vo ? make_int2(vo + j, vis_img[vo + j]) : make_int2(-1, -1);
    }
    if (is_target && k < n_targets) is_target[targets[k]] = stamp;
}
__global__ void setup_kernel(const double *__restrict__ vp, int S, SrcGeo *__restrict__ geo,
                             const int32_t *__restrict__ targets, int n_targets, const int32_t *__restrict__ vis_off,
                             const int32_t *__restrict__ vis_img, int M, int2 *__restrict__ items,
                             int32_t *__restrict__ is_target, int32_t stamp, int32_t *__restrict__ prep_mark,
                             const int64_t *__restrict__ nbr_off, const int32_t *__restrict__ nbr_idx,
                             const int32_t *__restrict__ live) {
    setup_thread(blockIdx.x * blockDim.x + threadIdx.x, vp, S, geo, targets, n_targets, vis_off, vis_img, M, items, is_target,
                 stamp, prep_mark, nbr_off, nbr_idx, live);
}

#define WORK_NT 256
#define WORK_CLASSES 4
__device__ inline void visit_chunks(int k, const int32_t *__restrict__ targets, const DevPatch *__restrict__ patches,
                                    const int32_t *__restrict__ vis_off, const int32_t *__restrict__ vis_img, int N, int M,
                                    int chunk_px, int G, bool dense, int &n_full, int &last_class, int *n_chunks = nullptr) {
    n_full = 0; last_class = 0;
    if (n_chunks) *n_chunks = 0;
    const int ti = k / M, j = k - ti * M;
    const int t = targets[ti];
    int n = j;
    if (!dense) {
        const int vo = vis_off[t];
        if (j >= vis_off[t + 1] - vo) return;
        n = vis_img[vo + j];
    }
    const DevPatch &P = patches[dense ? t * N + n : vis_off[t] + j];
    const int npx = P.H2 * P.W2;
    if (npx <= 0) return;
    if (n_chunks) *n_chunks = (npx + chunk_px - 1) / chunk_px;
    const int gpx = chunk_px * G;
    const int ngr = (npx + gpx - 1) / gpx;
    const int last_px = npx - (ngr - 1) * gpx;
    const int ipc = chunk_px >> 6;
    const int last_iters = (last_px / chunk_px) * ipc + ((last_px % chunk_px + 63) >> 6);
    const int shortfall = G * ipc - last_iters;
    last_class = shortfall == 0 ? 0 : 1 + ((shortfall - 1) * (WORK_CLASSES - 1)) / (G * ipc - 1);
    n_full = last_class == 0 ? ngr : ngr - 1;
}

__device__ inline int block_rank(bool pred, int *s_wave , int &total) {
    const unsigned long long m = __ballot(pred);
    const int lane = threadIdx.x & 63, wv = threadIdx.x >> 6;
    const int r = __popcll(m & ((1ull << lane) - 1ull));
    __syncthreads();
    if (lane == 0) s_wave[wv] = __popcll(m);
    __syncthreads();
    int off = 0, tot = 0;
#pragma unroll
    for (int w = 0; w < WORK_NT / 64; ++w) { const int c = s_wave[w]; off += w < wv ? c : 0; tot += c; }
    total = tot;
    return off + r;
}
__device__ inline int block_prefix(int v, int *s_wave , int &total) {
    const int lane = threadIdx.x & 63, wv = threadIdx.x >> 6;
    int x = v;
#pragma unroll
    for (int d = 1; d < 64; d <<= 1) { const int y = __shfl_up(x, d); if (lane >= d) x += y; }
    __syncthreads();
    if (lane == 63) s_wave[wv] = x;
    __syncthreads();
    int off = 0, tot = 0;
#pragma unroll
    for (int w = 0; w < WORK_NT / 64; ++w) { const int c = s_wave[w]; off += w < wv ? c : 0; tot += c; }
    total = tot;
    return off + x - v;
}

__global__ void __launch_bounds__(WORK_NT)
work_count_kernel(const int32_t *__restrict__ targets, int n_visits, const DevPatch *__restrict__ patches,
// ... 231 lines not shown
    const f2v *tp = reinterpret_cast<const f2v *>(tcf);
    const int n_dev = 8 * (NC / 14);
    for (int base = p0; base < p1; base += 128) {
        int h0[2], w0[2];
        bool ok[2];
        float dxs[2], dys[2], xh[2], xw[2];
#pragma unroll
        for (int q = 0; q < 2; ++q) {
            const int i = base + 64 * q + lane;
            ok[q] = i < p1;
            int rw, rh;
            divmod_small(min(i, p1 - 1), RH, rRH, rw, rh);
            h0[q] = h_lo + rh; w0[q] = w_lo + rw;
            const double hh = (double)(h0[q] + 1), ww = (double)(w0[q] + 1);
            dxs[q] = (float)(hh - si.m1); dys[q] = (float)(ww - si.m2);
            xh[q] = (float)(hh + sh0); xw[q] = (float)(ww + sw0);
        }
        const f2v dx = {dxs[0], dxs[1]}, dy = {dys[0], dys[1]};
        f2v f1 = (f2v)(0.0f);
        for (int c0 = 0; c0 < NC; c0 += (c0 < n_dev ? 8 : 6)) {
            const int len = c0 < n_dev ? 8 : 6;
            const f2v *k0 = tp + 3 * c0;
            const f2v d1 = dx - k0[3].xx, d2 = dy - k0[4].xx;
            const f2v s11 = -0.72134752044448170368f * (d1 * d1), s12 = -1.44269504088896340736f * (d1 * d2),
                      s22 = -0.72134752044448170368f * (d2 * d2);
            for (int c = c0; c < c0 + len; c += 2) {
                const f2v *k = tp + 3 * c;
                {
                    const f2v p11 = k[0].xx, p12 = k[1].xx, p22 = k[2].xx, w = k[5].xx;
                    const f2v q2 = p11 * s11 + (p12 * s12 + p22 * s22);
                    f1 += w * (f2v){__builtin_amdgcn_exp2f(q2.x), __builtin_amdgcn_exp2f(q2.y)};
                }
                {
#if CELESTE_MUTANT == 6
                    const f2v p11 = k[0].yy, p12 = k[1].xx, p22 = k[2].yy, w = k[5].yy;
#else
                    const f2v p11 = k[0].yy, p12 = k[1].yy, p22 = k[2].yy, w = k[5].yy;
#endif
                    const f2v q2 = p11 * s11 + (p12 * s12 + p22 * s22);
                    f1 += w * (f2v){__builtin_amdgcn_exp2f(q2.x), __builtin_amdgcn_exp2f(q2.y)};
                }
            }
        }
        const float *cc[2];
        float fxs[2], fys[2];
#pragma unroll
        for (int q = 0; q < 2; ++q) {
            int ix = (int)floorf(xh[q]); ix = ix < 1 ? 1 : (ix > 50 ? 50 : ix);
            int iy = (int)floorf(xw[q]); iy = iy < 1 ? 1 : (iy > 50 ? 50 : iy);
            cc[q] = coef + (ix - 1) + CEL_COEF * (iy - 1);
            fxs[q] = xh[q] - (float)ix; fys[q] = xw[q] - (float)iy;
        }
        f2v wx[4], wy[4];
        bspline_w((f2v){fxs[0], fxs[1]}, wx); bspline_w((f2v){fys[0], fys[1]}, wy);
        f2v y = (f2v)(0.0f);
#pragma unroll
        for (int b = 0; b < 4; ++b) {
            const float *ca = cc[0] + CEL_COEF * b, *cb = cc[1] + CEL_COEF * b;
            const f2v r = (f2v){ca[0], cb[0]} * wx[0] + (f2v){ca[1], cb[1]} * wx[1] + (f2v){ca[2], cb[2]} * wx[2] + (f2v){ca[3], cb[3]} * wx[3];
            y += r * wy[b];
        }
        const float f0s[2] = {y.x < 0 ? 1e-3f * __expf(y.x) : 1e-3f * (y.x + 1.0f), y.y < 0 ? 1e-3f * __expf(y.y) : 1e-3f * (y.y + 1.0f)};
        const float f1s[2] = {f1.x, f1.y};
#pragma unroll
        for (int q = 0; q < 2; ++q) {
            if (!ok[q]) continue;
            const double f0 = (double)f0s[q], g1 = (double)f1s[q];
            const double En = si.c0 * f0 + si.c1 * g1;
            const double E2n = si.q0 * (f0 * f0) + si.q1 * (g1 * g1);
            out[(h0[q] - P.off_h) + (int64_t)P.H2 * (w0[q] - P.off_w)] = make_double2(En, E2n - En * En);
        }
    }
}

#ifdef VALUE_TIMING
__device__ unsigned long long g_value_clk[8];
#endif
template <typename R, int WAVES = 1>
__global__ void __launch_bounds__(64 * WAVES)
value_kernel(const DevPatch *__restrict__ patches, const double *__restrict__ coefs,
             const SrcImg *__restrict__ srcimg, const Comp *__restrict__ comps,
             const int32_t *__restrict__ is_target, int32_t stamp, const int64_t *__restrict__ val_off,
             const int4 *__restrict__ items, int NC, int chunk_px, double2 *__restrict__ val,
             const float *__restrict__ coefs_f) {
    __shared__ double etab[64];
#ifdef VALUE_TIMING
    long long vts[4]; vts[0] = clock64();
#define VT(k) do { vts[(k) + 1] = clock64(); } while (0)
#else
#define VT(k) do { } while (0)
#endif
    const int4 it = items[blockIdx.x];
    const int sn = it.x, ch = it.z, t = it.w;
    if (is_target[t] != stamp) return;
    const DevPatch &P = patches[sn];
    const DevPatch &T = patches[it.y];
    const int h_lo = max(P.off_h, T.off_h), h_hi = min(P.off_h + P.H2, T.off_h + T.H2);
    const int w_lo = max(P.off_w, T.off_w), w_hi = min(P.off_w + P.W2 - 1, T.off_w + T.W2);
    const int RH = h_hi - h_lo, RW = w_hi - w_lo;
    if (RH <= 0 || RW <= 0) return;
    const int npx = RH * RW;
    const int p0 = ch * chunk_px;
    if (p0 >= npx) return;
    VT(0);
    exp_table_init(etab);
    const int p1 = min(npx, p0 + chunk_px);
    const SrcImg si = srcimg[sn];
    __shared__ Comp tc[14 * CEL_MAXK];
    {
        const double *src = reinterpret_cast<const double *>(comps + (size_t)sn * NC);
        double *dst = reinterpret_cast<double *>(tc);
        for (int i = threadIdx.x; i < NC * 8; i += 64 * WAVES) dst[i] = src[i];
        __syncthreads();
    }
    __shared__ float tcf[sizeof(R) == 4 ? 6 * 14 * CEL_MAXK : 2];
    if constexpr (sizeof(R) == 4) {
        if ((int)threadIdx.x < NC) {
            const Comp k = tc[threadIdx.x];
            float *o = tcf + 12 * (threadIdx.x >> 1) + (threadIdx.x & 1);
            o[0] = (float)k.p11; o[2] = (float)k.p12; o[4] = (float)k.p22; o[6] = (float)k.xi1; o[8] = (float)k.xi2; o[10] = (float)k.w0;
        }
        __syncthreads();
    }
    VT(1);
    if constexpr (sizeof(R) == 4) {
        const int q0 = p0 + 128 * (int)(threadIdx.x >> 6);
        if (WAVES == 1 || q0 < p1)
            value_pixels_f2(threadIdx.x & 63, P, si, NC, coefs_f + (size_t)(CELESTE_MUTANT == 3 ? 0 : P.stamp) * (CEL_COEF * CEL_COEF), h_lo, w_lo, RH,
                            WAVES == 1 ? p0 : q0, WAVES == 1 ? p1 : min(p1, q0 + 128), val + val_off[sn], tcf);
    } else if constexpr (WAVES == 1)
        value_pixels<false, R>(threadIdx.x, P, si, tc, NC, coefs, etab, h_lo, w_lo, RH, p0, p1, val + val_off[sn], tcf);
    else {
        const int q0 = p0 + 64 * (int)(threadIdx.x >> 6);
        if (q0 < p1) value_pixels<false, R>(threadIdx.x & 63, P, si, tc, NC, coefs, etab, h_lo, w_lo, RH, q0, min(p1, q0 + 64), val + val_off[sn], tcf);
    }
    VT(2);
#ifdef VALUE_TIMING
    if (threadIdx.x == 0) {
        for (int k = 0; k < 3; ++k) atomicAdd(&g_value_clk[k], (unsigned long long)(vts[k + 1] - vts[k]));
        atomicAdd(&g_value_clk[7], 1ull); atomicAdd(&g_value_clk[6], (unsigned long long)((p1 - p0 + 63) / 64));
    }
#endif
#undef VT
}

template <typename S>
struct PixelTermsT {
    typedef S scalar;
    S vterm, cnt_act, cnt_inact;
    S f0, f1;
    S alpha, beta, w2, w12;
    S k0, k1;
    S f0g0, f0g1, f0h0, f0h1, f0h2;
    S C0s, C0g, C1s, C1g;
    S Q0s, Q0g, Q1s, Q1g;
    S Wgg, Wsg, Wss;
    S S0d, S1x, S1y, S1xd, S1yd, S2a, S2b, S2c, S2an, S2bn, S2cn, S2ad, S2bd, S2cd;
    S S3a, S3b, S3c, S3d, S4a, S4b, S4c, S4d, S4e;
};
typedef PixelTermsT<double> PixelTerms;

template <int G, class TT>
__device__ __forceinline__ typename TT::scalar gal_g(const TT &T) {
    typedef typename TT::scalar S;
    if constexpr (G == 0) return T.S1x;
    else if constexpr (G == 1) return T.S1y;
    else if constexpr (G == 2) return T.S0d;
    else if constexpr (G == 3) return (S)0.5 * T.S2an;
    else if constexpr (G == 4) return T.S2bn;
    else return (S)0.5 * T.S2cn;
}
template <int G, int G2, class TT>
__device__ __forceinline__ typename TT::scalar gal_h(const TT &T) {
    typedef typename TT::scalar S;
    constexpr int k = G * 6 + G2;
// ... 1830 lines not shown
```

### celeste.jl_amd/csrc/group.h

```cpp
#pragma once
#include <rccl/rccl.h>
#include <chrono>
#include <condition_variable>
#include <functional>
#include <mutex>
#include <thread>

#define GROUP_MAX_MEMBERS 16
enum { GROUP_EXCHANGE_RCCL = 1, GROUP_EXCHANGE_PEER = 2 };

#define GROUP_ROW (CEL_P + 5)
#define GROUP_JROW (CEL_P + 1)

__global__ void group_pack_kernel(const double *__restrict__ vp, const int32_t *__restrict__ targets, int n,
                                  const int32_t *__restrict__ it, const int32_t *__restrict__ ev, const double *__restrict__ el,
                                  const int32_t *__restrict__ st, double *__restrict__ block, int row) {
    const int i = blockIdx.x, k = threadIdx.x;
    if (i >= n) return;
    const int t = targets[i];
    double *out = block + (size_t)i * row;
    const int head = row - CEL_P;
    if (k == 0) {
        out[0] = (double)t;
        if (head > 1) { out[1] = it ? (double)it[i] : 0.0; out[2] = ev ? (double)ev[i] : 0.0; out[3] = el ? el[i] : 0.0; out[4] = st ? (double)st[i] : 0.0; }
    }
    if (k < CEL_P) out[head + k] = vp[(size_t)t * CEL_P + k];
}

struct GroupCounts { int n[GROUP_MAX_MEMBERS]; };
__global__ void group_scatter_kernel(double *__restrict__ vp, const double *__restrict__ gathered, GroupCounts cnt, int n_members,
                                     int self, int width, int row) {
    const int j = blockIdx.y, i = blockIdx.x, k = threadIdx.x;
    if (j == self || j >= n_members || i >= cnt.n[j] || k >= CEL_P) return;
    const double *in = gathered + ((size_t)j * width + i) * row;
    const int t = (int)in[0];
    if (t < 0) return;
    vp[(size_t)t * CEL_P + k] = in[row - CEL_P + k];
}

struct GroupMember {
    int index = 0, device = 0;
    celeste_ctx *ctx = nullptr;
    ncclComm_t comm = nullptr;
    hipStream_t comm_stream = nullptr;
    hipEvent_t done[2] = {}, buf_free[2] = {}, t0 = nullptr, t1 = nullptr, t2 = nullptr;
    double *d_vp = nullptr, *d_vp_nbr = nullptr, *d_entry = nullptr;
    int32_t *d_targets = nullptr, *d_idx = nullptr;
    double *d_pos = nullptr;
    int32_t *d_it = nullptr, *d_ev = nullptr, *d_st = nullptr;
    double *d_el = nullptr;
    size_t tgt_cap = 0;
    double *d_block[2] = {nullptr, nullptr}, *d_gathered = nullptr, *d_h = nullptr;
    size_t block_cap = 0, gathered_cap = 0, h_cap = 0;
    double *p_gathered = nullptr, *p_h = nullptr;
    size_t p_gathered_cap = 0, p_h_cap = 0;
    std::vector<int32_t> idx;
    std::vector<int32_t> tg;
    int64_t n_chunks = 0;
    std::thread th;
    std::mutex mu;
    std::condition_variable cv;
    std::function<int()> task;
    bool has_task = false, quit = false;
    std::atomic<bool> busy{false};
    int result = CELESTE_OK;
    std::atomic<uint64_t> enq{0};
    std::atomic<int> in_coll{0}, in_wait{0};
};

struct celeste_group {
    int n = 0, n_devices = 0, exchange = 0, rccl_ranks = 0;
    int S = 0;
    std::vector<GroupMember *> mem;
    std::vector<celeste_images *> images;
    std::vector<int64_t> cost;
    double *p_vp = nullptr, *p_vp_nbr = nullptr;
    bool threads = false;
    std::mutex bmu; std::condition_variable bcv; int b_count = 0; uint64_t b_gen = 0; bool b_abort = false;
    int32_t plan_n = 0; uint32_t plan_flags = 0; int plan_width = 0; size_t plan_blk = 0; uint64_t sweep_k = 0; bool planned = false;
    bool timing = false;
    std::atomic<int> abort_rc{0};
    std::mutex call_mu;
    uint64_t enq_expected = 0;
    std::atomic<bool> need_abort{false}, force_abort{false}, broken{false};
    int64_t timeout_ms = 300000;
    int fault_member = -1, fault_site = 0, fault_delay_ms = 0;
    std::atomic<int> fault_nth{0};
};
enum { GROUP_FAULT_SWEEP = 1, GROUP_FAULT_ROWS = 2, GROUP_FAULT_BARRIER = 3, GROUP_FAULT_LAUNCH = 4 };
static bool group_fault(celeste_group *g, const GroupMember *m, int site) {
    if (g->fault_member != m->index || g->fault_site != site) return false;
    if (g->fault_nth.fetch_sub(1) != 1) return false;
    fprintf(stderr, "celeste_mi355x: injected fault (CELESTE_GROUP_FAULT): member %d, site %d\n", m->index, site);
    if (g->fault_delay_ms > 0) std::this_thread::sleep_for(std::chrono::milliseconds(g->fault_delay_ms));
    return true;
}

static bool group_barrier(celeste_group *g) {
    if (g->n <= 1) return true;
    std::unique_lock<std::mutex> lk(g->bmu);
    if (g->b_abort) return false;
    const uint64_t gen = g->b_gen;
    if (++g->b_count == g->n) { g->b_count = 0; ++g->b_gen; g->bcv.notify_all(); return true; }
    g->bcv.wait(lk, [&] { return g->b_gen != gen || g->b_abort; });
    return g->b_gen != gen;
}
static void group_fail(celeste_group *g) {
    std::lock_guard<std::mutex> lk(g->bmu);
    g->b_abort = true;
    g->bcv.notify_all();
}
static void group_barrier_reset(celeste_group *g) {
    std::lock_guard<std::mutex> lk(g->bmu);
    g->b_abort = false; g->b_count = 0;
}

static void group_worker(GroupMember *m) {
    (void)hipSetDevice(m->device);
    std::unique_lock<std::mutex> lk(m->mu);
    for (;;) {
        m->cv.wait(lk, [&] { return m->has_task || m->quit; });
        if (m->quit) return;
        std::function<int()> fn = std::move(m->task);
        m->has_task = false;
        lk.unlock();
        int r;
        try { r = fn(); } catch (const std::bad_alloc &) { r = CELESTE_ERR_ALLOC; } catch (...) { r = CELESTE_ERR_HIP; }
        lk.lock();
        if (m->result == CELESTE_OK) m->result = r;
        m->busy = false;
// ... 324 lines not shown
    }
    std::vector<int32_t> order(n);
    for (size_t i = 0; i < n; ++i) order[i] = (int32_t)i;
    std::stable_sort(order.begin(), order.end(), [&](int32_t a, int32_t b) { return weight[a] > weight[b]; });
    std::vector<int64_t> load((size_t)n_members, 0);
    shards.assign((size_t)n_members, {});
    for (int32_t i : order) {
        int k = 0;
        for (int p = 1; p < n_members; ++p) if (load[p] < load[k]) k = p;
        shards[k].push_back(i);
        load[k] += weight[i];
    }
    for (auto &s : shards) std::sort(s.begin(), s.end());
}

static int group_check_targets(celeste_group *g, int32_t n, const int32_t *targets) {
    if (n < 0 || (n > 0 && !targets)) return CELESTE_ERR_INVALID_ARG;
    for (int t = 0; t < n; ++t) if (targets[t] < 0 || targets[t] >= g->S) return CELESTE_ERR_INVALID_ARG;
    return CELESTE_OK;
}

static void group_shard(celeste_group *g, int32_t n, const int32_t *targets) {
    std::vector<int64_t> w((size_t)n);
    for (int t = 0; t < n; ++t) w[t] = g->cost[targets[t]];
    std::vector<std::vector<int32_t>> shards;
    group_lpt(g->n, w, shards);
    for (int r = 0; r < g->n; ++r) {
        GroupMember *m = g->mem[r];
        m->idx.swap(shards[r]);
        m->tg.resize(m->idx.size());
        m->n_chunks = 0;
        for (size_t i = 0; i < m->idx.size(); ++i) { m->tg[i] = targets[m->idx[i]]; m->n_chunks += m->ctx->h_src_chunks[m->tg[i]]; }
    }
}

static int group_target_buffers(GroupMember *m, size_t n) {
    if (n <= m->tgt_cap && m->d_targets) return CELESTE_OK;
    HIP_TRY(hipStreamSynchronize(m->ctx->stream));
    HIP_TRY(hipStreamSynchronize(m->comm_stream));
    void **ps[] = {(void **)&m->d_targets, (void **)&m->d_pos, (void **)&m->d_it, (void **)&m->d_ev, (void **)&m->d_st, (void **)&m->d_el,
                   (void **)&m->d_idx};
    const size_t by[] = {sizeof(int32_t), 2 * sizeof(double), sizeof(int32_t), sizeof(int32_t), sizeof(int32_t), sizeof(double), sizeof(int32_t)};
    m->tgt_cap = 0;
    for (int k = 0; k < 7; ++k) {
        if (*ps[k]) { (void)hipFree(*ps[k]); *ps[k] = nullptr; }
        HIP_TRY(hipMalloc(ps[k], std::max<size_t>(n, 1) * by[k]));
    }
    m->tgt_cap = std::max<size_t>(n, 1);
    return CELESTE_OK;
}

static inline size_t sweep_block_doubles(int W) { return (size_t)W * (1 + CEL_P + 2) + ((size_t)W + 1) / 2; }

static int group_quiesce(celeste_group *g) {
    int rc = group_join(g);
    for (GroupMember *m : g->mem) {
        if (!m->ctx) continue;
        int s1 = CELESTE_OK;
        if (hipSetDevice(m->device) != hipSuccess) { (void)hipGetLastError(); s1 = CELESTE_ERR_HIP; }
        if (s1 == CELESTE_OK) s1 = group_stream_wait(g, m, m->comm_stream, true);
        if (s1 == CELESTE_OK || s1 == CELESTE_ERR_ABORTED) { const int s2 = group_stream_wait(g, m, m->ctx->stream, true); if (s1 == CELESTE_OK) s1 = s2; }
        if (m->ctx->copy_stream && hipStreamSynchronize(m->ctx->copy_stream) != hipSuccess) { (void)hipGetLastError(); if (s1 == CELESTE_OK) s1 = CELESTE_ERR_HIP; }
        if (s1 != CELESTE_OK && rc == CELESTE_OK) rc = s1;
    }
    if (g->broken.load()) rc = CELESTE_ERR_ABORTED;
    return rc;
}

static int group_plan_locked(celeste_group *g, const double *vp, int32_t n_targets, const int32_t *targets, uint32_t flags, bool sync = true) {
    g->planned = false;
    (void)group_quiesce(g);
    if (g->broken.load()) return CELESTE_ERR_ABORTED;
    group_barrier_reset(g);
    group_shard(g, n_targets, targets);
    int W = 1;
    for (GroupMember *m : g->mem) W = std::max(W, (int)m->idx.size());
    g->plan_n = n_targets; g->plan_flags = flags; g->plan_width = W; g->plan_blk = sweep_block_doubles(W); g->sweep_k = 0;
    memcpy(g->p_vp, vp, (size_t)g->S * CEL_P * sizeof(double));
    const bool want_h = (flags & CELESTE_FLAG_HESS) != 0;
    const size_t HS = (flags & CELESTE_FLAG_PACKED_HESS) ? CELESTE_HP : (size_t)CEL_P * CEL_P;
    int rc = group_run(g, [&](GroupMember *m) -> int {
        HIP_TRY(hipSetDevice(m->device));
        hipStream_t st = m->ctx->stream;
        int s1 = group_target_buffers(m, m->tg.size());
        if (s1 != CELESTE_OK) return s1;
        const size_t blk = g->plan_blk;
        if (blk > m->block_cap) {
            HIP_TRY(hipStreamSynchronize(st)); HIP_TRY(hipStreamSynchronize(m->comm_stream));
            for (int k = 0; k < 2; ++k) { if (m->d_block[k]) (void)hipFree(m->d_block[k]); m->d_block[k] = nullptr; }
            m->block_cap = 0;
            for (int k = 0; k < 2; ++k) HIP_TRY(hipMalloc((void **)&m->d_block[k], blk * sizeof(double)));
            m->block_cap = blk;
        }
        for (int k = 0; k < 2; ++k) HIP_TRY(hipMemsetAsync(m->d_block[k], 0, blk * sizeof(double), st));
        s1 = group_grow(&m->d_gathered, &m->gathered_cap, blk * g->n, m->comm_stream);
        if (s1 == CELESTE_OK && want_h) s1 = group_grow(&m->d_h, &m->h_cap, std::max<size_t>(m->tg.size(), 1) * HS, st);
        if (s1 != CELESTE_OK) return s1;
        HIP_TRY(hipMemcpyAsync(m->d_vp, g->p_vp, (size_t)g->S * CEL_P * sizeof(double), hipMemcpyHostToDevice, st));
        if (!m->tg.empty()) {
            HIP_TRY(hipMemcpyAsync(m->d_targets, m->tg.data(), m->tg.size() * sizeof(int32_t), hipMemcpyHostToDevice, st));
            HIP_TRY(hipMemcpyAsync(m->d_idx, m->idx.data(), m->idx.size() * sizeof(int32_t), hipMemcpyHostToDevice, st));
        }
        for (int k = 0; k < 2; ++k) HIP_TRY(hipEventRecord(m->buf_free[k], st));
        if (sync) HIP_TRY(hipStreamSynchronize(st));
        return CELESTE_OK;
    });
    g->planned = rc == CELESTE_OK;
    return rc;
}

extern "C" int celeste_group_sweep_plan(celeste_group_t *g, const double *vp, int32_t n_targets, const int32_t *targets,
                                        uint32_t flags) try {
    if (!g || !vp || n_targets < 1 || (flags & (CELESTE_FLAG_SPLIT))) return CELESTE_ERR_INVALID_ARG;
    if (group_check_targets(g, n_targets, targets) != CELESTE_OK) return CELESTE_ERR_INVALID_ARG;
    std::lock_guard<std::mutex> lock(g->call_mu);
    return group_plan_locked(g, vp, n_targets, targets, flags);
} ABI_CATCH

static int group_sweep_member(celeste_group *g, GroupMember *m, int k) {
    HIP_TRY(hipSetDevice(m->device));
    hipStream_t st = m->ctx->stream;
    const int W = g->plan_width;
    double *blk = m->d_block[k];
    HIP_TRY(hipStreamWaitEvent(st, m->buf_free[k], 0));
    if (g->timing) HIP_TRY(hipEventRecord(m->t0, st));
    int own_rc = CELESTE_OK;
    if (group_fault(g, m, GROUP_FAULT_LAUNCH)) own_rc = CELESTE_ERR_HIP;
    else if (!m->tg.empty())
        own_rc = launch_eval(m->ctx, m->d_vp, (int32_t)m->tg.size(), m->d_targets, g->plan_flags, blk, blk + W, m->d_h,
                             reinterpret_cast<int64_t *>(blk + (size_t)W * (1 + CEL_P)),
                             reinterpret_cast<int32_t *>(blk + (size_t)W * (1 + CEL_P + 2)), st, true, nullptr, m->n_chunks);
    if (g->timing) HIP_TRY(hipEventRecord(m->t1, st));
    if (group_fault(g, m, GROUP_FAULT_SWEEP)) return CELESTE_ERR_HIP;
    HIP_TRY(hipEventRecord(m->done[k], st));
    HIP_TRY(hipStreamWaitEvent(m->comm_stream, m->done[k], 0));
    int rc = group_exchange(g, m, blk, g->plan_blk, m->comm_stream);
    if (rc != CELESTE_OK) return rc;
    HIP_TRY(hipEventRecord(m->buf_free[k], m->comm_stream));
    if (g->timing) HIP_TRY(hipEventRecord(m->t2, m->comm_stream));
    return own_rc;
}

extern "C" int celeste_group_sweep(celeste_group_t *g) try {
    if (!g) return CELESTE_ERR_INVALID_ARG;
    std::lock_guard<std::mutex> lock(g->call_mu);
    if (g->broken.load()) return CELESTE_ERR_ABORTED;
    if (!g->planned) return CELESTE_ERR_INVALID_ARG;
    const int k = (int)(g->sweep_k++ & 1);
    group_dispatch(g, [g, k](GroupMember *m) -> int { return group_sweep_member(g, m, k); }, 1);
    if (!g->threads) return group_join(g);
    return g->broken.load() ? CELESTE_ERR_ABORTED : CELESTE_OK;
} ABI_CATCH

extern "C" int celeste_group_sweep_wait(celeste_group_t *g) try {
    if (!g) return CELESTE_ERR_INVALID_ARG;
    std::lock_guard<std::mutex> lock(g->call_mu);
    return group_quiesce(g);
} ABI_CATCH

static int group_catalog_to_host(celeste_group *g, const double *p_gathered, uint32_t flags, double *v, double *d, int64_t *counters,
                                 int32_t *status) {
    const int W = g->plan_width;
    const size_t blk = g->plan_blk;
    const bool want_d = d && (flags & (CELESTE_FLAG_GRAD | CELESTE_FLAG_HESS));
    int worst = CELESTE_OK;
    for (int r = 0; r < g->n; ++r) {
        const GroupMember *o = g->mem[r];
        const double *b = p_gathered + (size_t)r * blk;
        const int64_t *bc = reinterpret_cast<const int64_t *>(b + (size_t)W * (1 + CEL_P));
        const int32_t *bs = reinterpret_cast<const int32_t *>(b + (size_t)W * (1 + CEL_P + 2));
        for (size_t i = 0; i < o->idx.size(); ++i) {
            const size_t q = (size_t)o->idx[i];
            if (v) v[q] = b[i];
            if (want_d) memcpy(d + q * CEL_P, b + W + i * CEL_P, CEL_P * sizeof(double));
            if (counters) { counters[2 * q] = bc[2 * i]; counters[2 * q + 1] = bc[2 * i + 1]; }
            if (status) status[q] = bs[i];
            if (bs[i] != CELESTE_OK && worst == CELESTE_OK) worst = bs[i];
        }
    }
    return worst;
}

static inline bool shard_contiguous(const GroupMember *m) { return !m->idx.empty() && (size_t)(m->idx.back() - m->idx.front()) + 1 == m->idx.size(); }
static int group_hessians_down(GroupMember *m, double *h, bool direct, size_t HS, size_t lo, size_t hi, hipStream_t stream) {
    if (hi <= lo) return CELESTE_OK;
    double *dst = direct ? h + ((size_t)m->idx[0] + lo) * HS : m->p_h + lo * HS;
    HIP_TRY(hipMemcpyAsync(dst, m->d_h + lo * HS, (hi - lo) * HS * sizeof(double), hipMemcpyDeviceToHost, stream));
    return CELESTE_OK;
}
static inline void group_hessians_scatter(const GroupMember *m, double *h, size_t HS, size_t lo, size_t hi) {
    for (size_t i = lo; i < hi; ++i) memcpy(h + (size_t)m->idx[i] * HS, m->p_h + i * HS, HS * sizeof(double));
}

static int group_results_locked(celeste_group *g, double *v, double *d, double *h, int64_t *counters, int32_t *status) {
    const size_t blk = g->plan_blk;
    const uint32_t flags = g->plan_flags;
    const bool want_h = h && (flags & CELESTE_FLAG_HESS);
    const size_t HS = (flags & CELESTE_FLAG_PACKED_HESS) ? CELESTE_HP : (size_t)CEL_P * CEL_P;
    const bool pin_h = want_h && is_pinned(h, (size_t)g->plan_n * HS * sizeof(double));
    int worst = CELESTE_OK;
    int rc = group_run(g, [&](GroupMember *m) -> int {
        HIP_TRY(hipSetDevice(m->device));
        hipStream_t st = m->ctx->stream;
        if (m->index == 0) {
            int s1 = group_grow_pinned(&m->p_gathered, &m->p_gathered_cap, blk * g->n);
            if (s1 != CELESTE_OK) return s1;
            HIP_TRY(hipMemcpyAsync(m->p_gathered, m->d_gathered, blk * g->n * sizeof(double), hipMemcpyDeviceToHost, st));
        }
        const size_t nr = m->tg.size();
        const bool direct = pin_h && shard_contiguous(m);
        int n_parts = 0;
        size_t part_lo[celeste_ctx::MAX_PARTS + 1] = {0};
        if (want_h && nr > 0) {
            if (!direct) { int s1 = group_grow_pinned(&m->p_h, &m->p_h_cap, nr * HS); if (s1 != CELESTE_OK) return s1; }
// ... 467 lines not shown
```

### celeste.jl_amd/elbo.py

```python
import time
import ctypes as C
from dataclasses import dataclass
from typing import Optional, Sequence

import numpy as np

from . import cabi
from .cabi import FLAG_GRAD, FLAG_HESS, FLAG_KL, P


@dataclass
class SensitiveFloat:
    v: float
    d: Optional[np.ndarray]
    h: Optional[np.ndarray]
    active_pixel_counter: int = 0
    inactive_pixel_counter: int = 0

    @property
    def has_gradient(self):
        return self.d is not None

    @property
    def has_hessian(self):
        return self.h is not None


class FieldContext:

    def __init__(self, images, patches, neighbors=None, psf_K: int = 2, prior: Optional[dict] = None,
                 device: int = 0, image_set: Optional["cabi.ImageSet"] = None, problem: Optional["cabi.Problem"] = None):
        self.lib = cabi.load_library()
        self.problem = problem if problem is not None else cabi.Problem(images, patches, neighbors, psf_K=psf_K, prior=prior,
                                                                        marshal_images=image_set is None)
        self.S, self.N = self.problem.n_sources, self.problem.n_images
        h = C.c_void_p()
        t0 = time.perf_counter()
        if image_set is None:
            self.device = device
            cabi.check(self.lib.celeste_ctx_create(C.byref(self.problem.c), device, C.byref(h)), self.lib)
        else:
            assert len(image_set.images) == self.N
            self.device = image_set.device
            cabi.check(self.lib.celeste_ctx_create_on(image_set.handle, C.byref(self.problem.c), C.byref(h)), self.lib)
        self.create_ms = (time.perf_counter() - t0) * 1e3
        self.handle = h

    @classmethod
    def from_catalog(cls, images, catalog, psf_K: int = 2, prior: Optional[dict] = None, device: int = 0,
                     image_set: Optional["cabi.ImageSet"] = None, sparse: Optional[bool] = None):
        from . import model
        if sparse is None:
            sparse = len(images) > 8
        table = model.patch_table(images, catalog, sparse=sparse)
        neighbors = table.neighbors()
        problem = cabi.problem_from_table(images, table, neighbors, psf_K=psf_K, prior=prior,
                                          marshal_images=image_set is None)
        ctx = cls(images, None, neighbors, psf_K=psf_K, prior=prior, device=device, image_set=image_set, problem=problem)
        ctx.table = table
        return ctx

    def close(self):
        if getattr(self, "_mcmc", None) is not None:
            self._mcmc.close()
            self._mcmc = None
        if getattr(self, "_blend", None) is not None:
            self._blend.close()
            self._blend = None
        if getattr(self, "handle", None):
            self.lib.celeste_ctx_destroy(self.handle)
            self.handle = None

    def mcmc_context(self):
        if getattr(self, "_mcmc", None) is None:
            from .mcmc import MCMCContext
            self._mcmc = MCMCContext(self.problem, self.device)
        return self._mcmc

    def blend_context(self):
        if getattr(self, "_blend", None) is None:
            from .blend import BlendContext
            self._blend = BlendContext(self.problem, self.device)
        return self._blend

    def mcmc_ais(self, catalog, targets: Sequence[int], cfg=None):
        from .mcmc import run_ais_batch
        return run_ais_batch(self, catalog, targets, cfg)

    def mcmc_loglike(self, catalog, targets: Sequence[int], model: int, which: Sequence[int], theta, boxes=None):
        from .mcmc import target_boxes
        mc = self.mcmc_context()
        if boxes is None:
            boxes = target_boxes(self.problem.images, catalog, targets)
        return mc.loglike(catalog, targets, boxes, model, which, theta)

    def __del__(self):
        try:
            self.close()
        except Exception:
            pass

    def eval_batch(self, vp, targets: Sequence[int], flags: int = FLAG_GRAD | FLAG_HESS | FLAG_KL,
                   raise_on_error: bool = True, pinned: bool = True):
        vp = np.ascontiguousarray(np.asarray(vp, dtype=np.float64).reshape(self.S, P))
        tg = np.ascontiguousarray(np.asarray(targets, dtype=np.int32))
        n = tg.size
        big = pinned and n >= 64
        v = np.zeros(n)
        d = np.zeros((n, P)) if flags & (FLAG_GRAD | FLAG_HESS) else None
        h = None
        if flags & FLAG_HESS:
            hshape = (n, cabi.HP) if flags & cabi.FLAG_PACKED_HESS else (n, P, P)
            h = cabi.pinned_empty(hshape) if big else np.zeros(hshape)
        cnt = np.zeros((n, 2), dtype=np.int64)
        status = np.zeros(n, dtype=np.int32)
        dp = cabi.c_double_p
        st = self.lib.celeste_elbo_eval_batch(
            self.handle, vp.ctypes.data_as(dp), n, tg.ctypes.data_as(cabi.c_int32_p), flags,
            v.ctypes.data_as(dp), d.ctypes.data_as(dp) if d is not None else None,
            h.ctypes.data_as(dp) if h is not None else None, cnt.ctypes.data_as(cabi.c_int64_p),
            status.ctypes.data_as(cabi.c_int32_p))
        if st in (cabi.ERR_NONFINITE_INPUT, cabi.ERR_NONFINITE_RESULT):
            if raise_on_error:
                raise AssertionError(self.lib.celeste_strerror(st).decode())
            bad = status != 0
            if d is not None:
                d[bad] = np.nan
            if h is not None:
                h[bad] = np.nan
        else:
            cabi.check(st, self.lib)
        return v, d, h, cnt, status

    def eval_multi(self, vp, active: Sequence[int], flags: int = FLAG_GRAD | FLAG_HESS | FLAG_KL):
        vp = np.ascontiguousarray(np.asarray(vp, dtype=np.float64).reshape(self.S, P))
        act = np.ascontiguousarray(np.asarray(active, dtype=np.int32))
        sa = act.size
        want_h = bool(flags & FLAG_HESS)
        want_d = want_h or bool(flags & FLAG_GRAD)
        v = C.c_double()
        d = np.zeros(sa * P) if want_d else None
        h = np.zeros((sa * P, sa * P)) if want_h else None
        na = C.c_int64(); ni = C.c_int64()
        dp = cabi.c_double_p
        st = self.lib.celeste_elbo_eval_multi(self.handle, vp.ctypes.data_as(dp), sa, act.ctypes.data_as(cabi.c_int32_p),
                                              flags, C.byref(v), d.ctypes.data_as(dp) if want_d else None,
                                              h.ctypes.data_as(dp) if want_h else None, C.byref(na), C.byref(ni))
        if st in (cabi.ERR_NONFINITE_INPUT, cabi.ERR_NONFINITE_RESULT):
            raise AssertionError(self.lib.celeste_strerror(st).decode())
        cabi.check(st, self.lib)
        return (v.value, d.reshape(sa, P).T.copy() if want_d else None, h, np.array([na.value, ni.value]))

    def eval_batch_device(self, d_vp: int, n_targets: int, d_targets: int, flags: int, d_v: int, d_d: int,
                          d_h: int, d_counters: int, d_status: int, stream: int = 0):
        cabi.check(self.lib.celeste_elbo_eval_batch_device(self.handle, d_vp, n_targets, d_targets, flags, d_v, d_d,
                                                           d_h, d_counters, d_status, stream), self.lib)

    def maximize_batch(self, vp, targets: Sequence[int], cfg: Optional["ElboConfig"] = None, include_kl: bool = True,
                       vp_neighbors=None, pos_centers=None, raise_on_error: bool = True):
        cfg = cfg or ElboConfig()
        vp = np.ascontiguousarray(np.asarray(vp, dtype=np.float64).reshape(self.S, P)).copy()
        tg = np.ascontiguousarray(np.asarray(targets, dtype=np.int32))
        n = tg.size
        its = np.zeros(n, dtype=np.int32); evals = np.zeros(n, dtype=np.int32)
        el = np.zeros(n); status = np.zeros(n, dtype=np.int32)
        ccfg = cfg.to_c(include_kl)
        nb = None if vp_neighbors is None else np.ascontiguousarray(
            np.asarray(vp_neighbors, dtype=np.float64).reshape(self.S, P))
        pc = None if pos_centers is None else np.ascontiguousarray(np.asarray(pos_centers, dtype=np.float64).reshape(n, 2))
        st = self.lib.celeste_maximize_batch(self.handle, vp.ctypes.data_as(cabi.c_double_p),
                                             nb.ctypes.data_as(cabi.c_double_p) if nb is not None else None,
                                             pc.ctypes.data_as(cabi.c_double_p) if pc is not None else None, n,
                                             tg.ctypes.data_as(cabi.c_int32_p), C.byref(ccfg),
                                             its.ctypes.data_as(cabi.c_int32_p), evals.ctypes.data_as(cabi.c_int32_p),
                                             el.ctypes.data_as(cabi.c_double_p), status.ctypes.data_as(cabi.c_int32_p))
        if st in (cabi.ERR_NONFINITE_INPUT, cabi.ERR_NONFINITE_RESULT):
            if raise_on_error:
                raise AssertionError(self.lib.celeste_strerror(st).decode())
        else:
            cabi.check(st, self.lib)
        return vp, its, evals, el, status

    def maximize_batch_device(self, d_vp: int, n_targets: int, d_targets: int, cfg: Optional["ElboConfig"] = None,
                              include_kl: bool = True, d_vp_neighbors: int = 0, d_pos_centers: int = 0, d_iterations: int = 0,
                              d_f_evals: int = 0, d_elbo: int = 0, d_status: int = 0, stream: int = 0):
        ccfg = (cfg or ElboConfig()).to_c(include_kl)
        cabi.check(self.lib.celeste_maximize_batch_device(self.handle, d_vp, d_vp_neighbors or None, d_pos_centers or None,
                                                          n_targets, d_targets, C.byref(ccfg), d_iterations or None,
                                                          d_f_evals or None, d_elbo or None, d_status or None, stream or None),
                   self.lib)

    def joint_infer(self, vp, layers: Sequence[Sequence[int]], cfg: Optional["ElboConfig"] = None, include_kl: bool = True,
                    pos_centers=None):
        cfg = cfg or ElboConfig()
        vp = np.ascontiguousarray(np.asarray(vp, dtype=np.float64).reshape(self.S, P)).copy()
        off = np.zeros(len(layers) + 1, dtype=np.int64)
        for l, layer in enumerate(layers):
            off[l + 1] = off[l] + len(layer)
        total = int(off[-1])
        tg = np.ascontiguousarray(np.concatenate([np.asarray(l, dtype=np.int32) for l in layers]) if total else np.zeros(0, np.int32))
        pc = None
        if pos_centers is not None:
            pc = np.ascontiguousarray(np.concatenate([np.asarray(c, dtype=np.float64).reshape(-1, 2) for c in pos_centers]))
            assert pc.shape == (total, 2)
        its = np.zeros(total, dtype=np.int32); evals = np.zeros(total, dtype=np.int32)
        el = np.zeros(total); status = np.zeros(total, dtype=np.int32)
        ccfg = cfg.to_c(include_kl)
        st = self.lib.celeste_joint_infer(self.handle, vp.ctypes.data_as(cabi.c_double_p), len(layers),
                                          off.ctypes.data_as(cabi.c_int64_p), tg.ctypes.data_as(cabi.c_int32_p),
                                          pc.ctypes.data_as(cabi.c_double_p) if pc is not None else None, C.byref(ccfg),
                                          its.ctypes.data_as(cabi.c_int32_p), evals.ctypes.data_as(cabi.c_int32_p),
                                          el.ctypes.data_as(cabi.c_double_p), status.ctypes.data_as(cabi.c_int32_p))
        if st not in (cabi.ERR_NONFINITE_INPUT, cabi.ERR_NONFINITE_RESULT):
            cabi.check(st, self.lib)
        return vp, its, evals, el, status

    def render_expected(self, vp, image: int) -> np.ndarray:
        vp = np.ascontiguousarray(np.asarray(vp, dtype=np.float64).reshape(self.S, P))
        img = self.problem.images[image]
        H, W = img.pixels.shape
        out = np.zeros(H * W)
        cabi.check(self.lib.celeste_render_expected(self.handle, vp.ctypes.data_as(cabi.c_double_p), image,
                                                    out.ctypes.data_as(cabi.c_double_p)), self.lib)
        return out.reshape(W, H).T.copy()

    def enable_timing(self, on: bool = True):
        cabi.check(self.lib.celeste_ctx_enable_timing(self.handle, 1 if on else 0), self.lib)

    def spline_coefficients(self, stamp: int) -> np.ndarray:
        out = np.empty(cabi.COEF * cabi.COEF)
        cabi.check(self.lib.celeste_ctx_spline_coefficients(self.handle, int(stamp), out.ctypes.data_as(cabi.c_double_p)), self.lib)
        return out.reshape(cabi.COEF, cabi.COEF).T.copy()

    def last_kernel_ms(self):
        ms = (C.c_float * 3)()
        cabi.check(self.lib.celeste_ctx_last_kernel_ms(self.handle, ms), self.lib)
        return [float(x) for x in ms]
# ... 86 lines not shown
```

### celeste.jl_amd/parallel.py

```python
from typing import Callable, Optional, Sequence, Tuple

import os

import numpy as np

from .partition import shard_targets

P = 44


def _default_all_gather(block: np.ndarray, world: int, device: Optional[int]):
    import torch
    import torch.distributed as dist
    if dist.get_backend() == "nccl":
        if device is None:
            raise ValueError("the nccl backend needs the device index of this rank's FieldContext (device=...)")
        t = torch.from_numpy(block).to("cuda:%d" % device)
    else:
        t = torch.from_numpy(block)
    outs = [torch.empty_like(t) for _ in range(world)]
    dist.all_gather(outs, t)
    return [o.cpu().numpy() for o in outs]


# ... 25 lines not shown

def sharded_maximize(maximize: Callable[[Sequence[int]], np.ndarray], targets: Sequence[int], costs: Sequence[float],
                     rank: int, world: int, all_gather: Optional[Callable] = None,
                     device: Optional[int] = None) -> np.ndarray:
    targets = list(targets)
    shards = shard_targets(costs, world)
    mine = [targets[i] for i in shards[rank]]
    res = maximize(mine) if mine else np.zeros((0, P))
    width = max(len(s) for s in shards)
    block = np.zeros((width, P))
    block[:len(mine)] = res
    if world == 1:
        blocks = [block]
    elif all_gather is not None:
        blocks = all_gather(block)
    else:
        blocks = _default_all_gather(block, world, device)
    out = np.zeros((len(targets), P))
    for r in range(world):
        out[shards[r]] = blocks[r][:len(shards[r])]
    return out


def gather_status(local_status: Sequence[int], n_targets: int, costs: Sequence[float], rank: int, world: int,
                  all_gather: Optional[Callable] = None, device: Optional[int] = None) -> np.ndarray:
    shards = shard_targets(costs, world)
    width = max(len(s) for s in shards)
    block = np.zeros((width, 1))
    block[:len(shards[rank]), 0] = np.asarray(local_status, dtype=np.float64)
    if world == 1:
        blocks = [block]
    elif all_gather is not None:
        blocks = all_gather(block)
    else:
        blocks = _default_all_gather(block, world, device)
    out = np.zeros(n_targets, dtype=np.int32)
    for r in range(world):
        out[shards[r]] = np.rint(blocks[r][:len(shards[r]), 0]).astype(np.int32)
    return out


class DeviceShardedSweep:

    def __init__(self, ctx, targets: Sequence[int], costs: Sequence[float], rank: int, world: int, flags: int,
                 backend: Optional[str] = None, shards=None):
        import torch
        self.torch = torch
        self.ctx, self.rank, self.world, self.flags = ctx, rank, world, flags
        self.targets = np.asarray(targets, dtype=np.int32)
        assert len(costs) == len(self.targets)
        self.shards = shards if shards is not None else shard_targets(costs, world)
        self.mine = self.targets[self.shards[rank]]
        self.n = int(self.mine.size)
        self.width = max(1, max(len(s) for s in self.shards))
        self.dev = torch.device("cuda", ctx.device)
        self.gather = world > 1
        if world == 1 and os.environ.get("CELESTE_GATHER_SINGLE") == "1":
            import torch.distributed as dist
            self.gather = dist.is_available() and dist.is_initialized()
        if self.gather:
            import torch.distributed as dist
            self.dist = dist
            self.backend = backend or dist.get_backend()
        else:
            self.backend = backend or "none"
        W = self.width
        with torch.cuda.device(self.dev):
            self.d_tg = torch.tensor(self.mine, dtype=torch.int32, device=self.dev)
            self.blocks = [torch.zeros(W * (1 + P), dtype=torch.float64, device=self.dev) for _ in range(2)]
            want_h = bool(flags & 2)
            self.d_h = torch.zeros(max(self.n, 1), P, P, dtype=torch.float64, device=self.dev) if want_h else None
            self.d_cnt = torch.zeros(max(self.n, 1), 2, dtype=torch.int64, device=self.dev)
            self.d_st = torch.zeros(max(self.n, 1), dtype=torch.int32, device=self.dev)
            self.compute_stream = torch.cuda.current_stream(self.dev)
            if self.gather and self.backend == "nccl":
                self.comm_stream = torch.cuda.Stream(self.dev)
                self.gathered = torch.zeros(world * W * (1 + P), dtype=torch.float64, device=self.dev)
                self.buf_free = [torch.cuda.Event(), torch.cuda.Event()]
                for e in self.buf_free:
                    e.record(self.compute_stream)
            elif self.gather:
                self.h_block = torch.zeros(W * (1 + P), dtype=torch.float64).pin_memory()
                self.gathered = torch.zeros(world * W * (1 + P), dtype=torch.float64)
        self.k = 0
        self.last = 0
        self.gather_bytes = world * W * (1 + P) * 8 if self.gather else 0

    def step(self, d_vp_ptr: int):
        torch = self.torch
        k = self.k & 1
        self.k += 1
        self.last = k
        blk = self.blocks[k]
        nccl = self.gather and self.backend == "nccl"
        if nccl:
            self.compute_stream.wait_event(self.buf_free[k])
        if self.n > 0:
            base = blk.data_ptr()
            self.ctx.eval_batch_device(d_vp_ptr, self.n, self.d_tg.data_ptr(), self.flags, base, base + 8 * self.width,
                                       self.d_h.data_ptr() if self.d_h is not None else 0, self.d_cnt.data_ptr(),
                                       self.d_st.data_ptr(), self.compute_stream.cuda_stream)
        if nccl:
            done = torch.cuda.Event()
            done.record(self.compute_stream)
            with torch.cuda.stream(self.comm_stream):
                self.comm_stream.wait_event(done)
                self.dist.all_gather_into_tensor(self.gathered, blk)
                self.buf_free[k].record(self.comm_stream)
        elif self.gather:
            self.h_block.copy_(blk, non_blocking=True)
            self.compute_stream.synchronize()
            outs = list(self.gathered.view(self.world, -1).unbind(0))
            self.dist.all_gather(outs, self.h_block)

    def wait(self):
        if self.gather and self.backend == "nccl":
            self.comm_stream.synchronize()
        self.torch.cuda.synchronize(self.dev)

    def results(self):
        self.wait()
        W = self.width
        g = (self.gathered if self.gather else self.blocks[self.last]).cpu().numpy().reshape(self.world, W * (1 + P))
        v = np.zeros(len(self.targets))
        d = np.zeros((len(self.targets), P))
        for r in range(self.world):
            idx = self.shards[r]
            v[idx] = g[r, :len(idx)]
            d[idx] = g[r, W:].reshape(W, P)[:len(idx)]
        return v, d, self.d_st[:self.n].cpu().numpy(), self.d_cnt[:self.n].cpu().numpy()

    def hessians(self):
        self.wait()
        return None if self.d_h is None else self.d_h[:self.n].cpu().numpy()


class DeviceJointInfer:

    def __init__(self, ctx, vp: np.ndarray, rank: int, world: int, cfg=None, backend: Optional[str] = None):
        import torch
        import torch.distributed as dist
        self.torch, self.dist = torch, dist
        self.ctx, self.rank, self.world, self.cfg = ctx, rank, world, cfg
        self.backend = backend or (dist.get_backend() if world > 1 else "none")
        self.dev = torch.device("cuda", ctx.device)
        with torch.cuda.device(self.dev):
            self.d_vp = torch.tensor(np.ascontiguousarray(vp, dtype=np.float64).reshape(ctx.S, P), device=self.dev)

    def layer(self, layer: Sequence[int], costs: Sequence[float], pos_centers: np.ndarray) -> np.ndarray:
        torch = self.torch
        layer = np.asarray(layer, dtype=np.int64)
        shards = shard_targets(costs, self.world)
        mine = shards[self.rank]
        W = max(1, max(len(s) for s in shards))
        with torch.cuda.device(self.dev):
            stream = torch.cuda.current_stream(self.dev)
            block = torch.zeros(W, P + 1, dtype=torch.float64, device=self.dev)
            if len(mine):
                d_tg = torch.tensor(layer[mine], dtype=torch.int32, device=self.dev)
                d_pc = torch.tensor(np.ascontiguousarray(pos_centers[mine], dtype=np.float64), device=self.dev)
                d_st = torch.zeros(len(mine), dtype=torch.int32, device=self.dev)
                self.ctx.maximize_batch_device(self.d_vp.data_ptr(), len(mine), d_tg.data_ptr(), self.cfg,
                                               d_pos_centers=d_pc.data_ptr(), d_status=d_st.data_ptr(),
                                               stream=stream.cuda_stream)
                block[:len(mine), :P] = self.d_vp[d_tg.long()]
                block[:len(mine), P] = d_st.double()
            if self.world == 1:
                gathered = block.unsqueeze(0)
            elif self.backend == "nccl":
# ... 22 lines not shown
```

### include/celeste_mi355x.h

```cpp
#ifndef CELESTE_MI355X_H
#define CELESTE_MI355X_H

#include <stddef.h>
#include <stdint.h>

#ifdef __cplusplus
extern "C" {
#endif

#define CELESTE_P 44
#define CELESTE_NUM_BANDS 5
#define CELESTE_STAMP 51
#define CELESTE_COEF 53
#define CELESTE_NUM_COLOR_COMPONENTS 8

enum {
    CELESTE_OK = 0,
    CELESTE_ERR_INVALID_ARG = 1,
    CELESTE_ERR_NONFINITE_INPUT = 2,
    CELESTE_ERR_NONFINITE_RESULT = 3,
    CELESTE_ERR_HIP = 4,
    CELESTE_ERR_NO_DEVICE = 5,
    CELESTE_ERR_ALLOC = 6,
    CELESTE_ERR_ABORTED = 7
};

enum {
    CELESTE_FLAG_GRAD = 1u,
    CELESTE_FLAG_HESS = 2u,
    CELESTE_FLAG_KL = 4u,
    CELESTE_FLAG_FP32 = 8u,
    CELESTE_FLAG_SPLIT = 16u,
    CELESTE_FLAG_PACKED_HESS = 32u
};
#define CELESTE_HP 990

typedef struct celeste_image_t {
    int32_t H;
    int32_t W;
    int32_t band;
    int32_t reserved;
    const float *pixels;
    const float *sky;
    const float *nelec_per_nmgy;
} celeste_image_t;

typedef struct celeste_patch_t {
    int32_t off_h;
    int32_t off_w;
    int32_t H2;
    int32_t W2;
    const uint8_t *bitmap;
    double wcs_jacobian[4];
    double world_center[2];
    double pixel_center[2];
    const double *psf;
    int32_t stamp;
    int32_t reserved;
} celeste_patch_t;

typedef struct celeste_prior_t {
    double is_star[2];
    double flux_mean[2];
    double flux_var[2];
    double k[2][8];
    double color_mean[2][8][4];
    double color_cov[2][8][16];
    double gal_radius_px_mean;
    double gal_radius_px_var;
} celeste_prior_t;

typedef struct celeste_problem_t {
    int32_t n_images;
    int32_t n_sources;
    int32_t psf_K;
    int32_t n_stamps;
    const celeste_image_t *images;
    const celeste_patch_t *patches;
    const double *stamps;
    const int64_t *nbr_offsets;
    const int32_t *nbr_index;
    const celeste_prior_t *prior;
    int64_t n_patch_entries;
    const int32_t *patch_source;
    const int32_t *patch_image;
} celeste_problem_t;

typedef struct celeste_ctx celeste_ctx_t;
typedef struct celeste_images celeste_images_t;

typedef struct celeste_work_stats_t {
    int64_t n_targets;
    int64_t active_pixel_visits;
    int64_t patch_rows;
    int64_t neighbor_links;
    int64_t algorithmic_bytes;
    int64_t record_bytes;
    int64_t record_tiles;
} celeste_work_stats_t;

#define CELESTE_ABI_VERSION 220
int celeste_version(void);
const char *celeste_strerror(int status);

int celeste_ctx_create(const celeste_problem_t *problem, int device, celeste_ctx_t **out);
void celeste_ctx_destroy(celeste_ctx_t *ctx);

int celeste_images_create(int32_t n_images, const celeste_image_t *images, int device, celeste_images_t **out);
void celeste_images_destroy(celeste_images_t *images);
int celeste_ctx_create_on(celeste_images_t *images, const celeste_problem_t *problem, celeste_ctx_t **out);


void *celeste_host_alloc(size_t bytes);
void celeste_host_free(void *ptr);
int celeste_host_register(void *ptr, size_t bytes);
int celeste_host_unregister(void *ptr);

int celeste_elbo_eval(celeste_ctx_t *ctx, const double *vp, int32_t target, uint32_t flags,
                      double *v, double *d, double *h,
                      int64_t *n_active_px, int64_t *n_inactive_px);

int celeste_elbo_eval_batch(celeste_ctx_t *ctx, const double *vp, int32_t n_targets,
                            const int32_t *targets, uint32_t flags,
                            double *v, double *d, double *h,
                            int64_t *counters, int32_t *status);

int celeste_elbo_eval_multi(celeste_ctx_t *ctx, const double *vp, int32_t n_active, const int32_t *active,
                            uint32_t flags, double *v, double *d, double *h,
                            int64_t *n_active_px, int64_t *n_inactive_px);

int celeste_elbo_eval_batch_device(celeste_ctx_t *ctx, const double *d_vp, int32_t n_targets,
                                   const int32_t *d_targets, uint32_t flags,
                                   double *d_v, double *d_d, double *d_h,
                                   int64_t *d_counters, int32_t *d_status, void *stream);

int celeste_ctx_enable_timing(celeste_ctx_t *ctx, int enable);
int celeste_ctx_last_kernel_ms(celeste_ctx_t *ctx, float ms[3]);
int celeste_ctx_last_record_sum_ms(celeste_ctx_t *ctx, float *ms);

int celeste_ctx_work_stats(celeste_ctx_t *ctx, int32_t n_targets, const int32_t *targets,
                           celeste_work_stats_t *out);

int celeste_spline_prefilter(const double *stamp51, double *coef53);
int celeste_ctx_spline_coefficients(celeste_ctx_t *ctx, int32_t stamp, double *coef53);

int celeste_psf_raster(int device, const double *psf, int32_t K,
                       const double *rows, int32_t n_rows,
                       const double *cols, int32_t n_cols, double *out);

typedef struct celeste_optim_config_t {
    double loc_width;
    double loc_scale;
    int32_t max_iters;
    int32_t include_kl;
    double xtol_abs;
    double ftol_rel;
    double gtol;
    double initial_delta;
    double delta_hat;
    int32_t tr_secular_iters;
    int32_t reserved;
} celeste_optim_config_t;

int celeste_maximize_batch(celeste_ctx_t *ctx, double *vp, const double *vp_neighbors, const double *pos_centers,
                           int32_t n_targets, const int32_t *targets, const celeste_optim_config_t *cfg,
                           int32_t *iterations, int32_t *f_evals, double *elbo, int32_t *status);

int celeste_maximize_batch_device(celeste_ctx_t *ctx, double *d_vp, const double *d_vp_neighbors,
                                  const double *d_pos_centers, int32_t n_targets, const int32_t *d_targets,
                                  const celeste_optim_config_t *cfg, int32_t *d_iterations, int32_t *d_f_evals,
                                  double *d_elbo, int32_t *d_status, void *stream);

int celeste_joint_infer(celeste_ctx_t *ctx, double *vp, int32_t n_layers, const int64_t *layer_offsets,
                        const int32_t *layer_targets, const double *pos_centers, const celeste_optim_config_t *cfg,
                        int32_t *iterations, int32_t *f_evals, double *elbo, int32_t *status);

int celeste_optim_stats(int reset, uint64_t out[5]);

#define CELESTE_NF 41
int celeste_tr_solve_batch(int device, int32_t n, const double *H, const double *g, const double *delta,
                           int32_t solver, int32_t secular_iters, double *p, double *m, int32_t *interior,
                           int32_t *fell_back);

int celeste_render_expected(celeste_ctx_t *ctx, const double *vp, int32_t image, double *out_plane);

typedef struct celeste_group celeste_group_t;
enum { CELESTE_EXCHANGE_RCCL = 1, CELESTE_EXCHANGE_PEER_COPY = 2 };
typedef struct celeste_group_info_t {
    int32_t n_members;
    int32_t n_devices;
    int32_t exchange;
    int32_t rccl_ranks;
    int32_t devices[16];
} celeste_group_info_t;
int celeste_group_create(const celeste_problem_t *problem, int32_t n_members, const int32_t *devices, celeste_group_t **out);
void celeste_group_destroy(celeste_group_t *group);
int celeste_group_info(celeste_group_t *group, celeste_group_info_t *out);
int celeste_group_collectives(celeste_group_t *group, int64_t *enqueued, int32_t *aborted);

int celeste_group_elbo_eval_batch(celeste_group_t *group, const double *vp, int32_t n_targets, const int32_t *targets,
                                  uint32_t flags, double *v, double *d, double *h, int64_t *counters, int32_t *status);

int celeste_group_sweep_plan(celeste_group_t *group, const double *vp, int32_t n_targets, const int32_t *targets, uint32_t flags);
int celeste_group_sweep(celeste_group_t *group);
int celeste_group_sweep_wait(celeste_group_t *group);
int celeste_group_sweep_results(celeste_group_t *group, double *v, double *d, double *h, int64_t *counters, int32_t *status);
int celeste_group_shard_sizes(celeste_group_t *group, int32_t *sizes, int64_t *costs);
int celeste_group_enable_timing(celeste_group_t *group, int enable);
int celeste_group_last_sweep_ms(celeste_group_t *group, float *eval_ms, float *gather_ms);
int celeste_group_last_kernel_ms(celeste_group_t *group, int32_t member, float ms[3]);

int celeste_group_maximize_batch(celeste_group_t *group, double *vp, const double *vp_neighbors, const double *pos_centers,
                                 int32_t n_targets, const int32_t *targets, const celeste_optim_config_t *cfg,
                                 int32_t *iterations, int32_t *f_evals, double *elbo, int32_t *status);

int celeste_group_joint_infer(celeste_group_t *group, double *vp, int32_t n_sweeps, int32_t n_batches,
                              const int64_t *batch_offsets, const int64_t *comp_offsets, const int32_t *comp_targets,
// ... 8 lines not shown
```

Baseline: 3.070 million sources/sec.

## Add prepared target lists that precompute work schedules for repeated evaluations

Adds a celeste_targets object that builds the per-target work decomposition once: setup, work count/scan/fill, needed marks, visit and value-item lists. Later evaluations on the same target set launch only geo_prep, value and pixel kernels, restricted to the relevant visits and value items. The aim is to cut per-call planning kernels and the device-to-host readback of the work total. The path is used by the parallel stepper and group sweeps. The trade-off is extra device memory per list and falling back to the old path when fused eval applies.

```diff
diff --git a/__graft_entry__.py b/__graft_entry__.py
--- a/__graft_entry__.py
+++ b/__graft_entry__.py
@@ -28,6 +28,7 @@
 def build() -> None:
     srcs = [os.path.join(CSRC, f) for f in os.listdir(CSRC) if f.endswith((".hip", ".h", ".inc", ".map"))]
     srcs.append(os.path.join(ROOT, "include", "celeste_mi355x.h"))
+    srcs.append(os.path.join(ROOT, "include", "celeste_targets.h"))
     srcs.append(os.path.abspath(__file__))
     if _stale(LIB, srcs):
         subprocess.check_call([HIPCC] + HIP_FLAGS + ["-o", LIB, os.path.join(CSRC, "celeste_abi.hip")] + LINK_FLAGS, cwd=CSRC)
@@ -46,6 +47,7 @@
     bsrcs = [os.path.join(BLEND_DIR, f) for f in os.listdir(BLEND_DIR) if f.endswith((".hip", ".h", ".map"))]
     bsrcs += [os.path.join(CSRC, f) for f in os.listdir(CSRC) if f.endswith((".hip", ".h", ".inc"))]
     bsrcs += [os.path.join(ROOT, "include", "celeste_blend.h"), os.path.join(ROOT, "include", "celeste_mi355x.h"),
+              os.path.join(ROOT, "include", "celeste_targets.h"),
               os.path.abspath(__file__)]
     if _stale(BLEND_LIB, bsrcs):
         subprocess.check_call([HIPCC] + HIP_FLAGS + ["-o", BLEND_LIB, os.path.join(BLEND_DIR, "celeste_blend.hip")] + LINK_FLAGS,
diff --git a/celeste.jl_amd/cabi.py b/celeste.jl_amd/cabi.py
--- a/celeste.jl_amd/cabi.py
+++ b/celeste.jl_amd/cabi.py
@@ -88,8 +88,9 @@
     "celeste_group_sweep_plan", "celeste_group_sweep", "celeste_group_sweep_wait", "celeste_group_sweep_results",
     "celeste_group_shard_sizes", "celeste_group_enable_timing", "celeste_group_last_sweep_ms", "celeste_group_last_kernel_ms",
     "celeste_group_maximize_batch", "celeste_group_joint_infer", "celeste_group_collectives",
+    "celeste_targets_create", "celeste_targets_create_device", "celeste_targets_destroy", "celeste_elbo_eval_targets_device",
 ]
-ABI_VERSION = 220
+ABI_VERSION = 221
 
 _lib = None
 
@@ -127,6 +128,11 @@
     lib.celeste_elbo_eval_batch.argtypes = [vp, c_double_p, C.c_int32, c_int32_p, C.c_uint32, c_double_p,
                                             c_double_p, c_double_p, c_int64_p, c_int32_p]
     lib.celeste_elbo_eval_batch_device.argtypes = [vp, vp, C.c_int32, vp, C.c_uint32, vp, vp, vp, vp, vp, vp]
+    lib.celeste_targets_create.argtypes = [vp, C.c_int32, c_int32_p, C.POINTER(vp)]
+    lib.celeste_targets_create_device.argtypes = [vp, C.c_int32, vp, vp, C.POINTER(vp)]
+    lib.celeste_targets_destroy.argtypes = [vp]
+    lib.celeste_targets_destroy.restype = None
+    lib.celeste_elbo_eval_targets_device.argtypes = [vp, vp, vp, C.c_uint32, vp, vp, vp, vp, vp, vp]
     lib.celeste_ctx_enable_timing.argtypes = [vp, C.c_int]
     lib.celeste_ctx_last_kernel_ms.argtypes = [vp, C.POINTER(C.c_float)]
     lib.celeste_elbo_eval_multi.argtypes = [vp, c_double_p, C.c_int32, c_int32_p, C.c_uint32, C.POINTER(C.c_double),
diff --git a/celeste.jl_amd/csrc/celeste_abi.hip b/celeste.jl_amd/csrc/celeste_abi.hip
--- a/celeste.jl_amd/csrc/celeste_abi.hip
+++ b/celeste.jl_amd/csrc/celeste_abi.hip
@@ -155,7 +155,9 @@
     int4 *d_vitems_src = nullptr;
     int32_t *d_vitem_off = nullptr;
     std::vector<int32_t> h_vitem_off;
+    std::vector<int32_t> h_vitem_tgt;
     int64_t n_value_items = 0;
+    std::vector<struct celeste_targets *> lists;
     int32_t *d_prep_mark = nullptr;
     double *d_lg_sum = nullptr;
     int64_t *d_nv_base = nullptr;
@@ -599,6 +601,8 @@
                 desc.push_back(make_int4((int)hv(s2, n), (int)hv(t, n), ch, t));
             }
         c->n_value_items = (int64_t)desc.size();
+        c->h_vitem_tgt.resize(desc.size());
+        for (size_t i = 0; i < desc.size(); ++i) c->h_vitem_tgt[i] = desc[i].w;
         CTX_TRY(dev_upload(&c->d_value_items, desc.data(), desc.size()));
         c->h_vitem_off.assign((size_t)c->S + 1, 0);
         for (auto &d : desc) c->h_vitem_off[(size_t)d.w + 1]++;
@@ -630,11 +634,14 @@
     return CELESTE_OK;
 } ABI_CATCH
 
+static void targets_free(struct celeste_targets *t);
 extern "C" void celeste_ctx_destroy(celeste_ctx_t *c) {
     if (!c) return;
     (void)hipSetDevice(c->device);
     if (c->stream) (void)hipStreamSynchronize(c->stream);
     if (c->copy_stream) (void)hipStreamSynchronize(c->copy_stream);
+    for (struct celeste_targets *t : c->lists) targets_free(t);
+    c->lists.clear();
     void *ptrs[] = {c->d_patches, c->d_coefs, c->d_coefs_f, c->d_bitmaps, c->d_nbr_off, c->d_nbr_idx, c->d_prior,
                     c->d_srcimg, c->d_comps, c->d_geo, c->d_val_off, c->d_val, c->d_needed, c->d_vis_off, c->d_vis_img, c->d_vis_src, c->d_value_items, c->d_vitems_src, c->d_vitem_off, c->d_prep_mark, c->d_rec_off, c->d_lg_sum, c->d_nv_base, c->d_nbr_vis, c->d_items, c->d_work, c->d_work_blk, c->d_work_total, c->d_tile_off, c->d_rec, c->d_acc_split, c->d_acc, c->d_vp, c->d_targets, c->d_v, c->d_d, c->d_h,
                     c->d_cnt, c->d_status};
@@ -738,6 +745,20 @@
 }
 
 #define VALUE_WIDE_MAX 768
+static bool want_eval_fused(uint32_t flags, int32_t n_targets, bool plain, const double *d_d, const double *d_h) {
+    const bool can = plain && (flags & CELESTE_FLAG_HESS) && !(flags & (CELESTE_FLAG_FP32 | CELESTE_FLAG_SPLIT)) && d_d && d_h;
+    bool eval_fused = can && n_targets <= EVAL_FUSED_MAX;
+    if (const char *e = getenv("CELESTE_EVAL_FUSED")) {
+        if (atoi(e) == 0) eval_fused = false;
+        else if (atoi(e) == 1) eval_fused = can;
+    }
+    return eval_fused;
+}
+static int chunk_group(int32_t n_targets) {
+    int G = n_targets >= 8192 ? 4 : n_targets >= 768 ? 2 : 1;
+    if (const char *e = getenv("CELESTE_CHUNK_GROUP")) if (atoi(e) >= 1 && atoi(e) <= 16) G = atoi(e);
+    return G;
+}
 static int launch_eval(celeste_ctx_t *c, const double *d_vp, int32_t n_targets, const int32_t *d_targets,
                        uint32_t flags, double *d_v, double *d_d, double *d_h, int64_t *d_counters, int32_t *d_status,
                        void *stream_, bool render_neighbors, const int32_t *d_active_rank, int64_t n_chunks,
@@ -781,15 +802,8 @@
         HIP_TRY(hipMalloc((void **)&c->d_work, std::max<size_t>(work_need, 1) * sizeof(int32_t)));
         c->work_cap = work_need;
     }
-    int G = n_targets >= 8192 ? 4 : n_targets >= 768 ? 2 : 1;
-    if (const char *e = getenv("CELESTE_CHUNK_GROUP")) if (atoi(e) >= 1 && atoi(e) <= 16) G = atoi(e);
-    bool eval_fused = !render_only && (flags & CELESTE_FLAG_HESS) && !(flags & (CELESTE_FLAG_FP32 | CELESTE_FLAG_SPLIT)) &&
-                      !d_active_rank && !d_live && !d_h_pos && d_d && d_h && n_targets <= EVAL_FUSED_MAX;
-    if (const char *e = getenv("CELESTE_EVAL_FUSED")) {
-        if (atoi(e) == 0) eval_fused = false;
-        else if (atoi(e) == 1) eval_fused = !render_only && (flags & CELESTE_FLAG_HESS) && !(flags & (CELESTE_FLAG_FP32 | CELESTE_FLAG_SPLIT)) &&
-                                          !d_active_rank && !d_live && !d_h_pos && d_d && d_h;
-    }
+    int G = chunk_group(n_targets);
+    const bool eval_fused = want_eval_fused(flags, n_targets, !render_only && !d_active_rank && !d_live && !d_h_pos, d_d, d_h);
     if (eval_fused) G = 1;
     const int n_classes = WORK_CLASSES;
     if ((size_t)n_wblk * (n_classes + 1) > c->work_blk_cap) {
@@ -948,6 +962,189 @@
     HIP_TRY(hipGetLastError());
     return CELESTE_OK;
 }
+
+struct celeste_targets {
+    celeste_ctx_t *ctx = nullptr;
+    int32_t n = 0;
+    int G = 1;
+    int32_t *d_targets = nullptr;
+    int32_t *d_work = nullptr, *d_work_total = nullptr, *d_rec_off = nullptr;
+    int2 *d_items = nullptr;
+    int32_t *d_needed = nullptr;
+    int32_t *d_visits = nullptr;
+    int32_t *d_vitems = nullptr;
+    int64_t n_visits = 0, n_vitems = 0;
+    int64_t n_records = 0;
+    int32_t n_work = 0;
+};
+static const int32_t LIST_STAMP = 1;
+
+static void targets_free(celeste_targets *t) {
+    if (!t) return;
+    void *ptrs[] = {t->d_targets, t->d_work, t->d_work_total, t->d_rec_off, t->d_items, t->d_needed, t->d_visits, t->d_vitems};
+    for (void *p : ptrs) if (p) (void)hipFree(p);
+    delete t;
+}
+
+static int targets_build(celeste_ctx_t *c, const std::vector<int32_t> &tg, celeste_targets_t **out) {
+    const int32_t n = (int32_t)tg.size();
+    if ((size_t)n * c->M * c->CH > 0x7fffffffull) return CELESTE_ERR_INVALID_ARG;
+    HIP_TRY(hipSetDevice(c->device));
+    celeste_targets *t = new celeste_targets;
+    t->ctx = c; t->n = n; t->G = chunk_group(n);
+    int32_t *d_blk = nullptr;
+    auto fail = [&](int st) { if (d_blk) (void)hipFree(d_blk); (void)hipGetLastError(); targets_free(t); return st; };
+#define LIST_TRY(expr) do { if ((expr) != hipSuccess) return fail(CELESTE_ERR_HIP); } while (0)
+#define LIST_ALLOC(p, bytes) do { if (hipMalloc((void **)&(p), (bytes)) != hipSuccess) return fail(CELESTE_ERR_ALLOC); } while (0)
+    std::vector<char> is_tgt((size_t)c->S, 0), reads((size_t)c->S, 0);
+    for (int32_t s : tg) {
+        is_tgt[s] = 1; reads[s] = 1;
+        for (int64_t q = c->h_nbr_off[s]; q < c->h_nbr_off[s + 1]; ++q) reads[c->h_nbr_idx[q]] = 1;
+        t->n_records += c->h_src_chunks[s];
+    }
+    std::vector<int32_t> visits, vitems;
+    for (int s = 0; s < c->S; ++s)
+        if (reads[s]) for (int v = c->h_vis_off[s]; v < c->h_vis_off[s + 1]; ++v) visits.push_back(v);
+    for (size_t i = 0; i < c->h_vitem_tgt.size(); ++i) if (is_tgt[c->h_vitem_tgt[i]]) vitems.push_back((int32_t)i);
+    t->n_visits = (int64_t)visits.size(); t->n_vitems = (int64_t)vitems.size();
+    const int n_cand = n * c->M;
+    const int n_wblk = (n_cand + WORK_NT - 1) / WORK_NT;
+    const size_t n_blk = (size_t)n_wblk * (WORK_CLASSES + 1);
+    LIST_ALLOC(t->d_targets, (size_t)n * sizeof(int32_t));
+    LIST_ALLOC(t->d_work, std::max<size_t>((size_t)t->n_records, 1) * sizeof(int32_t));
+    LIST_ALLOC(t->d_work_total, sizeof(int32_t));
+    LIST_ALLOC(t->d_rec_off, (size_t)n_cand * sizeof(int32_t));
+    if (!c->dense) LIST_ALLOC(t->d_items, (size_t)n_cand * sizeof(int2));
+    LIST_ALLOC(t->d_needed, (size_t)c->S * sizeof(int32_t));
+    LIST_ALLOC(t->d_visits, std::max<size_t>(visits.size(), 1) * sizeof(int32_t));
+    LIST_ALLOC(t->d_vitems, std::max<size_t>(vitems.size(), 1) * sizeof(int32_t));
+    LIST_ALLOC(d_blk, n_blk * sizeof(int32_t));
+    LIST_TRY(hipMemcpy(t->d_targets, tg.data(), (size_t)n * sizeof(int32_t), hipMemcpyHostToDevice));
+    if (!visits.empty()) LIST_TRY(hipMemcpy(t->d_visits, visits.data(), visits.size() * sizeof(int32_t), hipMemcpyHostToDevice));
+    if (!vitems.empty()) LIST_TRY(hipMemcpy(t->d_vitems, vitems.data(), vitems.size() * sizeof(int32_t), hipMemcpyHostToDevice));
+    LIST_TRY(hipMemset(t->d_needed, 0, (size_t)c->S * sizeof(int32_t)));
+    const size_t setup_threads = (size_t)n * (c->dense ? 1 : c->M);
+    hipLaunchKernelGGL(setup_kernel, dim3((unsigned)((setup_threads + 63) / 64)), dim3(64), 0, nullptr, (const double *)nullptr, -1,
+                       (SrcGeo *)nullptr, t->d_targets, n, c->d_vis_off, c->d_vis_img, c->M, t->d_items, t->d_needed, LIST_STAMP,
+                       (int32_t *)nullptr, c->d_nbr_off, c->d_nbr_idx, (const int32_t *)nullptr);
+    hipLaunchKernelGGL(work_count_kernel, dim3(n_wblk), dim3(WORK_NT), 0, nullptr, t->d_targets, n_cand, c->d_patches,
+                       c->d_vis_off, c->d_vis_img, c->N, c->M, c->chunk_px, t->G, (int)c->dense, d_blk, (const int32_t *)nullptr);
+    hipLaunchKernelGGL(work_scan_kernel, dim3(1), dim3(1024), 0, nullptr, d_blk, (int)n_blk, t->d_work_total, n_wblk * WORK_CLASSES);
+    hipLaunchKernelGGL(work_fill_kernel, dim3(n_wblk), dim3(WORK_NT), 0, nullptr, t->d_targets, n_cand, c->d_patches,
+                       c->d_vis_off, c->d_vis_img, c->N, c->M, c->CH, c->chunk_px, t->G, (int)c->dense, d_blk, t->d_work,
+                       (const int32_t *)nullptr, t->d_rec_off);
+    LIST_TRY(hipGetLastError());
+    LIST_TRY(hipMemcpy(&t->n_work, t->d_work_total, sizeof(int32_t), hipMemcpyDeviceToHost));
+    LIST_TRY(hipFree(d_blk)); d_blk = nullptr;
+#undef LIST_TRY
+#undef LIST_ALLOC
+    if (t->n_work < 0 || (int64_t)t->n_work > t->n_records) return fail(CELESTE_ERR_HIP);
+    c->lists.push_back(t);
+    *out = t;
+    return CELESTE_OK;
+}
+
+extern "C" int celeste_targets_create(celeste_ctx_t *c, int32_t n_targets, const int32_t *targets, celeste_targets_t **out) try {
+    if (!c || !out || !targets || n_targets <= 0) return CELESTE_ERR_INVALID_ARG;
+    *out = nullptr;
+    for (int32_t i = 0; i < n_targets; ++i) if (targets[i] < 0 || targets[i] >= c->S) return CELESTE_ERR_INVALID_ARG;
+    return targets_build(c, std::vector<int32_t>(targets, targets + n_targets), out);
+} ABI_CATCH
+
+extern "C" int celeste_targets_create_device(celeste_ctx_t *c, int32_t n_targets, const int32_t *d_targets, void *stream_,
+                                             celeste_targets_t **out) try {
+    if (!c || !out || !d_targets || n_targets <= 0) return CELESTE_ERR_INVALID_ARG;
+    *out = nullptr;
+    HIP_TRY(hipSetDevice(c->device));
+    std::vector<int32_t> tg((size_t)n_targets);
+    HIP_TRY(hipMemcpyAsync(tg.data(), d_targets, (size_t)n_targets * sizeof(int32_t), hipMemcpyDeviceToHost, (hipStream_t)stream_));
+    HIP_TRY(hipStreamSynchronize((hipStream_t)stream_));
+    for (int32_t s : tg) if (s < 0 || s >= c->S) return CELESTE_ERR_INVALID_ARG;
+    return targets_build(c, tg, out);
+} ABI_CATCH
+
+static void targets_release(celeste_targets_t *t) {
+    celeste_ctx_t *c = t->ctx;
+    auto it = std::find(c->lists.begin(), c->lists.end(), t);
+    if (it != c->lists.end()) c->lists.erase(it);
+    targets_free(t);
+}
+
+extern "C" void celeste_targets_destroy(celeste_targets_t *t) {
+    if (!t) return;
+    (void)hipSetDevice(t->ctx->device);
+    (void)hipDeviceSynchronize();
+    targets_release(t);
+}
+
+static int launch_prepared(celeste_ctx_t *c, const celeste_targets_t *t, const double *d_vp, uint32_t flags, double *d_v,
+                           double *d_d, double *d_h, int64_t *d_counters, int32_t *d_status, void *stream_) {
+    if (!c || !t || t->ctx != c) return CELESTE_ERR_INVALID_ARG;
+    const int32_t n_targets = t->n;
+    const char *off = getenv("CELESTE_NO_PREPARED");
+    if ((off && atoi(off) != 0) || (flags & (CELESTE_FLAG_FP32 | CELESTE_FLAG_SPLIT)) ||
+        want_eval_fused(flags, n_targets, true, d_d, d_h))
+        return launch_eval(c, d_vp, n_targets, t->d_targets, flags, d_v, d_d, d_h, d_counters, d_status, stream_, true, nullptr,
+                           t->n_records);
+    if (!d_vp || !d_v || !d_status) return CELESTE_ERR_INVALID_ARG;
+    if ((flags & CELESTE_FLAG_HESS) && !d_h) return CELESTE_ERR_INVALID_ARG;
+    if ((flags & (CELESTE_FLAG_GRAD | CELESTE_FLAG_HESS)) && !d_d) return CELESTE_ERR_INVALID_ARG;
+    hipStream_t stream = (hipStream_t)stream_;
+    HIP_TRY(hipSetDevice(c->device));
+    const size_t need = std::max<size_t>((size_t)t->n_records, 1) * ACC_N;
+    if (need > c->acc_cap) {
+        if (c->d_acc) { HIP_TRY(hipStreamSynchronize(stream)); HIP_TRY(hipFree(c->d_acc)); c->d_acc = nullptr; }
+        HIP_TRY(hipMalloc((void **)&c->d_acc, need * sizeof(double)));
+        c->acc_cap = need;
+    }
+    const int CH = c->CH, chunk_px = c->chunk_px;
+    if (c->timing) HIP_TRY(hipEventRecord(c->ev[0], stream));
+    const unsigned geo_blocks = (unsigned)((c->S + 63) / 64);
+    hipLaunchKernelGGL(geo_prep_kernel, dim3(geo_blocks + (unsigned)t->n_visits), dim3(64), 0, stream, d_vp, c->d_images,
+                       c->d_patches, c->d_vis_src, c->d_vis_img, c->K, c->d_srcimg, c->d_comps, t->d_visits, (int)geo_blocks,
+                       c->S, c->d_geo);
+    if (t->n_vitems > 0) {
+        const bool wide_items = n_targets <= VALUE_WIDE_MAX && c->chunk_px == 256 && !getenv("CELESTE_NO_WIDE_VALUE");
+#define LAUNCH_VALUE(WAVES)                                                                                                 \
+        hipLaunchKernelGGL((value_kernel<double, WAVES>), dim3((unsigned)t->n_vitems), dim3(64 * WAVES), 0, stream,        \
+                           c->d_patches, c->d_coefs, c->d_srcimg, c->d_comps, t->d_needed, LIST_STAMP, c->d_val_off,        \
+                           c->d_value_items, c->NC, c->chunk_px, c->d_val, c->d_coefs_f, t->d_vitems)
+        if (wide_items) LAUNCH_VALUE(4); else LAUNCH_VALUE(1);
+#undef LAUNCH_VALUE
+    }
+    if (c->timing) HIP_TRY(hipEventRecord(c->ev[1], stream));
+    const dim3 grid((unsigned)std::max<int32_t>(t->n_work, 1));
+#define LAUNCH_PIXEL(MODE)                                                                                                  \
+    hipLaunchKernelGGL((pixel_kernel<MODE, double>), grid, dim3(64), 0, stream, c->d_images, c->d_patches, c->d_coefs,      \
+                       c->d_bitmaps, c->d_srcimg, c->d_comps, c->d_nbr_off, c->d_nbr_idx, c->d_val_off, c->d_val,           \
+                       t->d_targets, c->N, c->NC, CH, chunk_px, t->G, c->d_acc, c->d_tile_off, c->d_rec,                    \
+                       (const int32_t *)nullptr, t->d_items, c->M, t->d_work, t->d_work_total, c->d_nv_base, c->d_nbr_vis,  \
+                       t->d_rec_off, c->d_coefs_f)
+    if (flags & CELESTE_FLAG_HESS) LAUNCH_PIXEL(2);
+    else if (flags & CELESTE_FLAG_GRAD) LAUNCH_PIXEL(1);
+    else LAUNCH_PIXEL(0);
+#undef LAUNCH_PIXEL
+    if (c->timing) HIP_TRY(hipEventRecord(c->ev[2], stream));
+    c->ev_split = 0;
+    const int lift_nt = n_targets <= 1024 ? 512 : 256;
+    bool lift7 = n_targets > 4096;
+    if (const char *e = getenv("CELESTE_LIFT_WAVES")) lift7 = atoi(e) == 7;
+#define LIFT_ARGS dim3(n_targets), dim3(lift_nt), 0, stream, d_vp, c->d_images, c->d_patches, c->d_geo, c->d_nbr_off,       \
+                  c->d_nbr_idx, t->d_targets, c->d_acc, c->d_prior, c->d_vis_off, c->d_vis_img, c->N, c->M, CH, chunk_px,   \
+                  flags, d_v, d_d, d_h, d_counters, d_status, (const int32_t *)nullptr, c->d_lg_sum, t->d_rec_off, \
+                  (const int32_t *)nullptr
+    if (lift7) hipLaunchKernelGGL(lift_kernel<7>, LIFT_ARGS); else hipLaunchKernelGGL(lift_kernel<8>, LIFT_ARGS);
+#undef LIFT_ARGS
+    if (c->timing) { HIP_TRY(hipEventRecord(c->ev[3], stream)); c->ev_valid = 1; }
+    HIP_TRY(hipGetLastError());
+    return CELESTE_OK;
+}
+
+extern "C" int celeste_elbo_eval_targets_device(celeste_ctx_t *c, const celeste_targets_t *t, const double *d_vp, uint32_t flags,
+                                                double *d_v, double *d_d, double *d_h, int64_t *d_counters,
+                                                int32_t *d_status, void *stream_) try {
+    return launch_prepared(c, t, d_vp, flags, d_v, d_d, d_h, d_counters, d_status, stream_);
+} ABI_CATCH
 
 __global__ void spin_kernel(long long ticks) {
     const long long t0 = wall_clock64();
diff --git a/celeste.jl_amd/csrc/elbo_kernels.h b/celeste.jl_amd/csrc/elbo_kernels.h
--- a/celeste.jl_amd/csrc/elbo_kernels.h
+++ b/celeste.jl_amd/csrc/elbo_kernels.h
@@ -125,6 +125,7 @@
     brightness_moments_wave(c, vs, p, b, srcimg + sn);
 }
 
+__device__ inline void source_geo(const double *vp, int s, SrcGeo *geo);
 __global__ void __launch_bounds__(64)
 prep_kernel(const double *__restrict__ vp, const DevImage *__restrict__ images,
             const DevPatch *__restrict__ patches, const int32_t *__restrict__ vis_src,
@@ -152,6 +153,19 @@
         if (mark && mark[s] != stamp) return;
     }
     prep_visit(threadIdx.x, s, n, sn, vp, images, patches, K, srcimg, comps);
+}
+
+__global__ void __launch_bounds__(64)
+geo_prep_kernel(const double *__restrict__ vp, const DevImage *__restrict__ images, const DevPatch *__restrict__ patches,
+                const int32_t *__restrict__ vis_src, const int32_t *__restrict__ vis_img, int K, SrcImg *__restrict__ srcimg,
+                Comp *__restrict__ comps, const int32_t *__restrict__ visit_list, int geo_blocks, int S, SrcGeo *__restrict__ geo) {
+    if ((int)blockIdx.x < geo_blocks) {
+        const int k = blockIdx.x * 64 + threadIdx.x;
+        if (k < S) source_geo(vp, k, geo);
+        return;
+    }
+    const int sn = visit_list[(int)blockIdx.x - geo_blocks];
+    prep_visit(threadIdx.x, vis_src[sn], vis_img[sn], sn, vp, images, patches, K, srcimg, comps);
 }
 
 __device__ __forceinline__ void source_geo_values(const double *vs, SrcGeo *out) {
@@ -488,7 +502,8 @@
                                     const int64_t *__restrict__ nbr_off, const int32_t *__restrict__ nbr_idx,
                                     const int32_t *__restrict__ live = nullptr) {
     if (live) n_targets = min(n_targets, *live);
-    if (S < 0) { if (k < n_targets) source_geo(vp, targets[k], geo); }
+    if (!vp) { }
+    else if (S < 0) { if (k < n_targets) source_geo(vp, targets[k], geo); }
     else if (k < S) source_geo(vp, k, geo);
     if (prep_mark && k < n_targets) {
         const int t = targets[k];
@@ -886,7 +901,7 @@
              const SrcImg *__restrict__ srcimg, const Comp *__restrict__ comps,
              const int32_t *__restrict__ is_target, int32_t stamp, const int64_t *__restrict__ val_off,
              const int4 *__restrict__ items, int NC, int chunk_px, double2 *__restrict__ val,
-             const float *__restrict__ coefs_f) {
+             const float *__restrict__ coefs_f, const int32_t *__restrict__ item_list = nullptr) {
     __shared__ double etab[64];
 #ifdef VALUE_TIMING
     long long vts[4]; vts[0] = clock64();
@@ -894,7 +909,7 @@
 #else
 #define VT(k) do { } while (0)
 #endif
-    const int4 it = items[blockIdx.x];
+    const int4 it = items[item_list ? item_list[blockIdx.x] : blockIdx.x];
     const int sn = it.x, ch = it.z, t = it.w;
     if (is_target[t] != stamp) return;
     const DevPatch &P = patches[sn];
diff --git a/celeste.jl_amd/csrc/group.h b/celeste.jl_amd/csrc/group.h
--- a/celeste.jl_amd/csrc/group.h
+++ b/celeste.jl_amd/csrc/group.h
@@ -46,6 +46,7 @@
     hipEvent_t done[2] = {}, buf_free[2] = {}, t0 = nullptr, t1 = nullptr, t2 = nullptr;
     double *d_vp = nullptr, *d_vp_nbr = nullptr, *d_entry = nullptr;
     int32_t *d_targets = nullptr, *d_idx = nullptr;
+    celeste_targets_t *plan_list = nullptr;
     double *d_pos = nullptr;
     int32_t *d_it = nullptr, *d_ev = nullptr, *d_st = nullptr;
     double *d_el = nullptr;
@@ -536,6 +537,7 @@
     int rc = group_run(g, [&](GroupMember *m) -> int {
         HIP_TRY(hipSetDevice(m->device));
         hipStream_t st = m->ctx->stream;
+        if (m->plan_list) { targets_release(m->plan_list); m->plan_list = nullptr; }
         int s1 = group_target_buffers(m, m->tg.size());
         if (s1 != CELESTE_OK) return s1;
         const size_t blk = g->plan_blk;
@@ -568,7 +570,13 @@
     if (!g || !vp || n_targets < 1 || (flags & (CELESTE_FLAG_SPLIT))) return CELESTE_ERR_INVALID_ARG;
     if (group_check_targets(g, n_targets, targets) != CELESTE_OK) return CELESTE_ERR_INVALID_ARG;
     std::lock_guard<std::mutex> lock(g->call_mu);
-    return group_plan_locked(g, vp, n_targets, targets, flags);
+    int rc = group_plan_locked(g, vp, n_targets, targets, flags);
+    if (rc != CELESTE_OK) return rc;
+    rc = group_run(g, [&](GroupMember *m) -> int {
+        return m->tg.empty() || (flags & CELESTE_FLAG_FP32) ? CELESTE_OK : celeste_targets_create(m->ctx, (int32_t)m->tg.size(), m->tg.data(), &m->plan_list);
+    });
+    if (rc != CELESTE_OK) g->planned = false;
+    return rc;
 } ABI_CATCH
 
 static int group_sweep_member(celeste_group *g, GroupMember *m, int k) {
@@ -581,9 +589,13 @@
     int own_rc = CELESTE_OK;
     if (group_fault(g, m, GROUP_FAULT_LAUNCH)) own_rc = CELESTE_ERR_HIP;
     else if (!m->tg.empty())
-        own_rc = launch_eval(m->ctx, m->d_vp, (int32_t)m->tg.size(), m->d_targets, g->plan_flags, blk, blk + W, m->d_h,
-                             reinterpret_cast<int64_t *>(blk + (size_t)W * (1 + CEL_P)),
-                             reinterpret_cast<int32_t *>(blk + (size_t)W * (1 + CEL_P + 2)), st, true, nullptr, m->n_chunks);
+        own_rc = m->plan_list
+            ? launch_prepared(m->ctx, m->plan_list, m->d_vp, g->plan_flags, blk, blk + W, m->d_h,
+                              reinterpret_cast<int64_t *>(blk + (size_t)W * (1 + CEL_P)),
+                              reinterpret_cast<int32_t *>(blk + (size_t)W * (1 + CEL_P + 2)), st)
+            : launch_eval(m->ctx, m->d_vp, (int32_t)m->tg.size(), m->d_targets, g->plan_flags, blk, blk + W, m->d_h,
+                          reinterpret_cast<int64_t *>(blk + (size_t)W * (1 + CEL_P)),
+                          reinterpret_cast<int32_t *>(blk + (size_t)W * (1 + CEL_P + 2)), st, true, nullptr, m->n_chunks);
     if (g->timing) HIP_TRY(hipEventRecord(m->t1, st));
     if (group_fault(g, m, GROUP_FAULT_SWEEP)) return CELESTE_ERR_HIP;
     HIP_TRY(hipEventRecord(m->done[k], st));
diff --git a/celeste.jl_amd/elbo.py b/celeste.jl_amd/elbo.py
--- a/celeste.jl_amd/elbo.py
+++ b/celeste.jl_amd/elbo.py
@@ -45,6 +45,7 @@
             cabi.check(self.lib.celeste_ctx_create_on(image_set.handle, C.byref(self.problem.c), C.byref(h)), self.lib)
         self.create_ms = (time.perf_counter() - t0) * 1e3
         self.handle = h
+        self._prepared = {}
 
     @classmethod
     def from_catalog(cls, images, catalog, psf_K: int = 2, prior: Optional[dict] = None, device: int = 0,
@@ -68,6 +69,9 @@
             self._blend.close()
             self._blend = None
         if getattr(self, "handle", None):
+            for h in getattr(self, "_prepared", {}).values():
+                self.lib.celeste_targets_destroy(h)
+            self._prepared = {}
             self.lib.celeste_ctx_destroy(self.handle)
             self.handle = None
 
@@ -151,8 +155,30 @@
         cabi.check(st, self.lib)
         return (v.value, d.reshape(sa, P).T.copy() if want_d else None, h, np.array([na.value, ni.value]))
 
+    def prepare_targets(self, d_targets: int, n_targets: int, stream: int = 0):
+        key = (int(d_targets), int(n_targets))
+        self.forget_targets(*key)
+        h = C.c_void_p()
+        cabi.check(self.lib.celeste_targets_create_device(self.handle, n_targets, d_targets, stream, C.byref(h)), self.lib)
+        self._prepared[key] = h
+        return h
+
+    def forget_targets(self, d_targets: int, n_targets: int):
+        h = self._prepared.pop((int(d_targets), int(n_targets)), None)
+        if h is not None:
+            self.lib.celeste_targets_destroy(h)
+
+    def eval_targets_device(self, handle, d_vp: int, flags: int, d_v: int, d_d: int, d_h: int, d_counters: int,
+                            d_status: int, stream: int = 0):
+        cabi.check(self.lib.celeste_elbo_eval_targets_device(self.handle, handle, d_vp, flags, d_v, d_d, d_h, d_counters,
+                                                             d_status, stream), self.lib)
+
     def eval_batch_device(self, d_vp: int, n_targets: int, d_targets: int, flags: int, d_v: int, d_d: int,
                           d_h: int, d_counters: int, d_status: int, stream: int = 0):
+        if self._prepared:
+            h = self._prepared.get((int(d_targets), int(n_targets)))
+            if h is not None:
+                return self.eval_targets_device(h, d_vp, flags, d_v, d_d, d_h, d_counters, d_status, stream)
         cabi.check(self.lib.celeste_elbo_eval_batch_device(self.handle, d_vp, n_targets, d_targets, flags, d_v, d_d,
                                                            d_h, d_counters, d_status, stream), self.lib)
 
diff --git a/celeste.jl_amd/parallel.py b/celeste.jl_amd/parallel.py
--- a/celeste.jl_amd/parallel.py
+++ b/celeste.jl_amd/parallel.py
@@ -131,9 +131,21 @@
             elif self.gather:
                 self.h_block = torch.zeros(W * (1 + P), dtype=torch.float64).pin_memory()
                 self.gathered = torch.zeros(world * W * (1 + P), dtype=torch.float64)
+        if self.n > 0 and hasattr(ctx, "prepare_targets"):
+            ctx.prepare_targets(self.d_tg.data_ptr(), self.n, self.compute_stream.cuda_stream)
         self.k = 0
         self.last = 0
         self.gather_bytes = world * W * (1 + P) * 8 if self.gather else 0
+
+    def close(self):
+        if self.n > 0 and getattr(self.ctx, "handle", None) and hasattr(self.ctx, "forget_targets"):
+            self.ctx.forget_targets(self.d_tg.data_ptr(), self.n)
+
+    def __del__(self):
+        try:
+            self.close()
+        except Exception:
+            pass
 
     def step(self, d_vp_ptr: int):
         torch = self.torch
diff --git a/include/celeste_mi355x.h b/include/celeste_mi355x.h
--- a/include/celeste_mi355x.h
+++ b/include/celeste_mi355x.h
@@ -99,7 +99,7 @@
     int64_t record_tiles;
 } celeste_work_stats_t;
 
-#define CELESTE_ABI_VERSION 220
+#define CELESTE_ABI_VERSION 221
 int celeste_version(void);
 const char *celeste_strerror(int status);
 
@@ -133,6 +133,8 @@
                                    const int32_t *d_targets, uint32_t flags,
                                    double *d_v, double *d_d, double *d_h,
                                    int64_t *d_counters, int32_t *d_status, void *stream);
+
+#include "celeste_targets.h"
 
 int celeste_ctx_enable_timing(celeste_ctx_t *ctx, int enable);
 int celeste_ctx_last_kernel_ms(celeste_ctx_t *ctx, float ms[3]);
diff --git a/include/celeste_targets.h b/include/celeste_targets.h
--- /dev/null
+++ b/include/celeste_targets.h
@@ -0,0 +1,13 @@
+#ifndef CELESTE_TARGETS_H
+#define CELESTE_TARGETS_H
+
+typedef struct celeste_targets celeste_targets_t;
+int celeste_targets_create(celeste_ctx_t *ctx, int32_t n_targets, const int32_t *targets, celeste_targets_t **out);
+int celeste_targets_create_device(celeste_ctx_t *ctx, int32_t n_targets, const int32_t *d_targets, void *stream,
+                                  celeste_targets_t **out);
+void celeste_targets_destroy(celeste_targets_t *targets);
+int celeste_elbo_eval_targets_device(celeste_ctx_t *ctx, const celeste_targets_t *targets, const double *d_vp, uint32_t flags,
+                                     double *d_v, double *d_d, double *d_h, int64_t *d_counters, int32_t *d_status,
+                                     void *stream);
+
+#endif
```

New measurement: 3.141 million sources/sec (median of 6 runs). 2.3% higher.
